# GBATZOLIS/ID-diff

Measured on AMD Instinct MI355X. Metric: score-vector evals/sec (rows of S per second incl. the per-point spectrum), 32x32 ncsnpp, higher is better.
Workload: dtype f32 (3x3 convs: Winograd, fp32 transforms, contraction on pairs of fp16 values -- 22 significand bits, 3 products, fp32 accumulate (F(4,3) along the rows x 3 filter rows); 1x1/attention/dense contractions: fp32 operands split exactly into 3 bf16, 6 partial products, fp32 accumulate; the q/k/v projec

## Files before the change

id-diff_amd/_lib.py:

```python
import ctypes
import os
import subprocess
from typing import NamedTuple, Optional

import torch

_HERE = os.path.dirname(os.path.abspath(__file__))
_VARIANT = os.environ.get("IDIFF_LIB_VARIANT", "")
_LIB_PATH = os.path.join(_HERE, "csrc", f"libidiff_hip.{_VARIANT}.so" if _VARIANT else "libidiff_hip.so")
_lib = None

ACT = {None: 0, "none": 0, "linear": 0, "silu": 1, "swish": 1, "elu": 2, "relu": 3, "lrelu": 4}

c_i, c_i64, c_f, c_d, c_p = ctypes.c_int, ctypes.c_int64, ctypes.c_float, ctypes.c_double, ctypes.c_void_p


class Epilogue(ctypes.Structure):
    _fields_ = [("bias", c_p), ("rowbias", c_p), ("ld_rowbias", c_i64), ("rows_per_group", c_i), ("act", c_i),
                ("residual", c_p), ("ld_residual", c_i64), ("out_scale", c_f), ("rowscale", c_p), ("colstats", c_p)]


_SIGNATURES = {
    "idiff_abi_version": (c_i, []),
    "idiff_last_error": (ctypes.c_char_p, []),
    "idiff_source_stamp": (ctypes.c_char_p, []),
    "idiff_variant_flags": (ctypes.c_char_p, []),
    "idiff_set_option": (c_i, [ctypes.c_char_p, c_i]),
    "idiff_gemm_pairs_ok": (c_i, [c_i, c_i, c_i, c_i]),
    "idiff_gemm_pairs_scale_f32": (c_i, [c_p, c_i64, c_i, c_i, c_p, c_p]),
    "idiff_gemm_pairs_f32": (c_i, [c_p, c_i64, c_i64, c_p, c_i64, c_i64, c_p, c_i, c_p, c_p, c_i64, c_i64, c_i, c_i, c_i, c_i, c_p, c_p]),
    "idiff_pairs_act_scale_f32": (c_i, [c_p, c_i, c_i, c_p, c_i, c_i, c_i, c_i, c_p, c_p]),
    "idiff_gemm_pairs_2src_f32": (c_i, [c_p, c_p, c_i64, c_i, c_p, c_p, c_i64, c_p, c_p, c_i64, c_i, c_i, c_i, c_p, c_p]),
    "idiff_set_thread_option": (c_i, [ctypes.c_char_p, c_i, c_i]),
    "idiff_upfirdn2d_f32": (c_i, [c_p, c_p, c_p] + [c_i] * 14 + [c_p]),
    "idiff_upfirdn2d_route": (ctypes.c_char_p, [c_p, c_p] + [c_i] * 14),
    "idiff_upfirdn2d_gn_f32": (c_i, [c_p, c_p, c_p, c_i, c_p] + [c_i] * 14 + [c_p]),
    "idiff_upfirdn2d_gn_ok": (c_i, [c_p, c_p, c_i, c_p] + [c_i] * 14),
    "idiff_fused_bias_act_f32": (c_i, [c_p, c_p, c_p, c_p, c_i64, c_i, c_i, c_i, c_i, c_f, c_f, c_p]),
    "idiff_upfirdn2d_f16": (c_i, [c_p, c_p, c_p] + [c_i] * 14 + [c_p]),
    "idiff_upfirdn2d_f64": (c_i, [c_p, c_p, c_p] + [c_i] * 14 + [c_p]),
    "idiff_fused_bias_act_f16": (c_i, [c_p, c_p, c_p, c_p, c_i64, c_i, c_i, c_i, c_i, c_f, c_f, c_p]),
    "idiff_fused_bias_act_f64": (c_i, [c_p, c_p, c_p, c_p, c_i64, c_i, c_i, c_i, c_i, c_f, c_f, c_p]),
    "idiff_gemm_f32": (c_i, [c_p, c_i64, c_i64, c_p, c_i64, c_i64, c_p, c_i64, c_i64, c_i, c_i, c_i, c_i,
                             ctypes.POINTER(Epilogue), c_p]),
    "idiff_gemm_2src_f32": (c_i, [c_p, c_p, c_i64, c_i, c_p, c_i64, c_p, c_i64, c_i, c_i, c_i, ctypes.POINTER(Epilogue), c_p]),
    "idiff_conv2d_nhwc_f32": (c_i, [c_p, c_p, c_p] + [c_i] * 10 + [ctypes.POINTER(Epilogue), c_p]),
    "idiff_gemm_route": (ctypes.c_char_p, [c_p, c_i64, c_i64, c_p, c_i64, c_i64, c_p, c_i64, c_i64, c_i, c_i, c_i, c_i,
                                           ctypes.POINTER(Epilogue), c_i]),
    "idiff_conv2d_route": (ctypes.c_char_p, [c_p, c_p, c_p] + [c_i] * 10 + [ctypes.POINTER(Epilogue)]),
    "idiff_gemm_colstats_split": (c_i, [c_i, c_i, c_i, c_i64, c_i64, c_i]),
    "idiff_conv2d_colstats_split": (c_i, [c_i] * 10),
    "idiff_conv2d_winograd_ok": (c_i, [c_i] * 5),
    "idiff_winograd_weight_floats": (c_i64, [c_i, c_i]),
    "idiff_winograd_pack_f32": (c_i, [c_p, c_p, c_i, c_i, c_p]),
    "idiff_conv2d_winograd_f32": (c_i, [c_p, c_p, c_p] + [c_i] * 5 + [ctypes.POINTER(Epilogue), c_p]),
    "idiff_conv2d_winograd_colstats_split": (c_i, [c_i] * 5),
    "idiff_conv2d_winograd43_ok": (c_i, [c_i] * 5),
    "idiff_conv2d_winograd43_colstats_split": (c_i, [c_i] * 5),
    "idiff_winograd43_weight_floats": (c_i64, [c_i, c_i]),
    "idiff_winograd43_pack_f32": (c_i, [c_p, c_p, c_i, c_i, c_p]),
    "idiff_conv2d_winograd43_f32": (c_i, [c_p, c_p, c_p, c_i, c_i, c_i, c_i, c_i, ctypes.POINTER(Epilogue), c_p]),
    "idiff_conv2d_winograd43h_ok": (c_i, [c_i] * 5),
    "idiff_winograd43h_weight_floats": (c_i64, [c_i, c_i]),
    "idiff_winograd43h_pack_f32": (c_i, [c_p, c_p, c_i, c_i, c_p]),
    "idiff_conv2d_winograd43h_f32": (c_i, [c_p, c_p, c_p, c_i, c_i, c_i, c_i, c_i, ctypes.POINTER(Epilogue), c_p]),
    "idiff_conv2d_wino1d_ok": (c_i, [c_i] * 5),
    "idiff_conv2d_wino1d_colstats_split": (c_i, [c_i] * 5),
    "idiff_wino1d_weight_floats": (c_i64, [c_i, c_i]),
    "idiff_wino1d_pack_f32": (c_i, [c_p, c_p, c_i, c_i, c_p]),
    "idiff_conv2d_wino1d_f32": (c_i, [c_p, c_p, c_p, c_i, c_i, c_i, c_i, c_i, ctypes.POINTER(Epilogue), c_p]),
    "idiff_conv2d_wino1d_gn_ok": (c_i, [c_i] * 6),
    "idiff_conv2d_wino1d_normload_ok": (c_i, [c_i] * 5),
    "idiff_conv2d_wino1d_normload_f32": (c_i, [c_p, c_p, c_p, c_i, c_i, c_i, c_i, c_i, ctypes.POINTER(Epilogue), c_p, c_i, c_p]),
    "idiff_conv2d_wino1d_normload_2src_ok": (c_i, [c_i] * 6),
    "idiff_conv2d_wino1d_normload_2src_f32": (c_i, [c_p, c_i, c_p, c_i, c_p, c_p, c_i, c_i, c_i, c_i, ctypes.POINTER(Epilogue), c_p, c_i, c_p]),
    "idiff_groupnorm_coef_f32": (c_i, [c_p, c_i, c_i, c_p, c_i, c_i, c_i, c_i, c_i, c_f, c_p, c_p, c_p, c_p]),
    "idiff_conv2d_wino1d_gn_f32": (c_i, [c_p, c_p, c_p, c_i, c_i, c_i, c_i, c_i, ctypes.POINTER(Epilogue), c_i, c_p, c_p, c_f, c_i, c_p]),
    "idiff_conv2d_winograd_split_ok": (c_i, [c_i] * 5),
    "idiff_winograd_split_weight_floats": (c_i64, [c_i, c_i]),
    "idiff_winograd_pack_split_f32": (c_i, [c_p, c_p, c_i, c_i, c_p]),
    "idiff_conv2d_winograd_split_f32": (c_i, [c_p, c_p, c_p] + [c_i] * 5 + [ctypes.POINTER(Epilogue), c_p]),
    "idiff_groupnorm_finalize_f32": (c_i, [c_p, c_i, c_i, c_p, c_i, c_i, c_i, c_i, c_i, c_f, c_p, c_p]),
    "idiff_groupnorm_nsplit": (c_i, [c_i, c_i, c_i]),
    "idiff_groupnorm_stats_f32": (c_i, [c_p, c_i, c_p, c_i, c_i, c_i, c_i, c_f, c_p, c_p, c_p]),
    "idiff_groupnorm_apply_f32": (c_i, [c_p, c_i, c_p, c_i, c_i, c_i, c_i, c_p, c_p, c_p, c_p, c_i64, c_i, c_p, c_p]),
    "idiff_groupnorm_apply_colstats_f32": (c_i, [c_p, c_i, c_p, c_i, c_i, c_i, c_i, c_p, c_i, c_p, c_i, c_f, c_p, c_p, c_p, c_i64,
                                                 c_i, c_p, c_p]),
    "idiff_groupnorm_apply_route": (ctypes.c_char_p, [c_p, c_i, c_p, c_i, c_i, c_i, c_i, c_p, c_p, c_p, c_p]),
    "idiff_groupnorm_apply_colstats_route": (ctypes.c_char_p, [c_p, c_i, c_p, c_i, c_i, c_i, c_i, c_p, c_i, c_p, c_i, c_p, c_p, c_p]),
    "idiff_softmax_rows_f32": (c_i, [c_p, c_p, c_i64, c_i, c_f, c_p]),
    "idiff_softmax_rows_route": (ctypes.c_char_p, [c_p, c_p, c_i64, c_i, c_f]),
    "idiff_attention256_ok": (c_i, [c_i, c_i, c_i]),
    "idiff_attention256_f32": (c_i, [c_p, c_i64, c_p, c_p, c_p, c_p, c_p, c_i, c_i, c_i, c_f, c_p]),
    "idiff_attention_heads_ok": (c_i, [c_i, c_i, c_i, c_i]),
    "idiff_attention_heads_f32": (c_i, [c_p, c_i64, c_p, c_p, c_p, c_p, c_p, c_i, c_i, c_i, c_i, c_f, c_p]),
    "idiff_attention256_route": (ctypes.c_char_p, [c_p, c_i64, c_p, c_p, c_p, c_p, c_p, c_i, c_i, c_i]),
    "idiff_attention_heads_route": (ctypes.c_char_p, [c_p, c_i64, c_p, c_p, c_p, c_p, c_p, c_i, c_i, c_i, c_i]),
    "idiff_affine_act_f32": (c_i, [c_p, c_p, c_i64, c_f, c_f, c_i, c_p, c_i64, c_p]),
    "idiff_add_scale_f32": (c_i, [c_p, c_p, c_p, c_i64, c_f, c_p]),
    "idiff_affine_act_route": (ctypes.c_char_p, [c_p, c_p, c_i64, c_p, c_i64]),
    "idiff_add_scale_route": (ctypes.c_char_p, [c_p, c_p, c_p, c_i64]),
    "idiff_concat_cols_route": (ctypes.c_char_p, [c_p, c_i, c_p, c_i, c_p, c_i64]),
    "idiff_fourier_embed_f32": (c_i, [c_p, c_p, c_p, c_i, c_i, c_p]),
    "idiff_positional_embed_f32": (c_i, [c_p, c_p, c_i, c_i, c_f, c_i, c_p]),
    "idiff_concat_cols_f32": (c_i, [c_p, c_i, c_p, c_i, c_p, c_i64, c_p]),
    "idiff_nchw_to_nhwc_f32": (c_i, [c_p, c_p, c_i, c_i, c_i, c_i, c_f, c_f, c_p]),
    "idiff_nhwc_to_nchw_f32": (c_i, [c_p, c_p, c_i, c_i, c_i, c_i, c_p, c_p]),
    "idiff_resample2x_nhwc_f32": (c_i, [c_p, c_p, c_i, c_i, c_i, c_i, c_i, c_p]),
    "idiff_perturb_f32": (c_i, [c_p, c_p, c_p, c_p, c_p, c_i64, c_i64, c_p]),
    "idiff_perturb_randn_f32": (c_i, [c_p, c_p, c_p, c_p, c_i64, c_i64, c_i64, ctypes.c_uint64, c_p, c_p]),
    "idiff_spectrum_workspace_bytes": (c_i64, [c_i, c_i, c_i]),
    "idiff_spectrum_f32": (c_i, [c_p, c_i, c_i, c_i, c_p, c_i64, c_p, c_p, c_p]),
    "idiff_colmean_f64": (c_i, [c_p, c_i, c_i, c_i, c_p, c_p, c_p]),
    "idiff_centered_gram_f64": (c_i, [c_p, c_p, c_i, c_i, c_i, c_p, c_p]),
    "idiff_centered_gram_rows_f64": (c_i, [c_p, c_p, c_i, c_i, c_i, c_i, c_p, c_p]),
    "idiff_symmetrize_upper_f64": (c_i, [c_p, c_i, c_p]),
    "idiff_symtridiag_scratch_doubles": (c_i64, [c_i]),
    "idiff_symband_ld": (c_i, []),
    "idiff_symband_f64": (c_i, [c_p, c_i, c_p, c_p]),
    "idiff_symtridiag_f64": (c_i, [c_p, c_i, c_i, c_p, c_p, c_p, c_p]),
    "idiff_symtridiag_plan": (c_i, [c_i]),
    "idiff_tridiag_eigvals_f64": (c_i, [c_p, c_p, c_i, c_i, c_p, c_p]),
    "idiff_sym_lowvecs_scratch_doubles": (c_i64, [c_i, c_i]),
    "idiff_sym_lowvecs_f64": (c_i, [c_p, c_i, c_i, c_p, c_p, c_p, c_p, c_p]),
    "idiff_sym_topvecs_scratch_doubles": (c_i64, [c_i, c_i, c_i]),
    "idiff_sym_topvecs_f64": (c_i, [c_p, c_i, c_i, c_i, c_d, c_d, c_d, c_i, c_i, c_p, c_p, c_p, c_p, c_p]),
    "idiff_knn_workspace_bytes": (c_i64, [c_i, c_i, c_i]),
    "idiff_knn_f32": (c_i, [c_p, c_i, c_i, c_i, c_p, c_i64, c_p, c_p, c_p, c_p]),
# ... 300 lines not shown
def gemm_pairs_ok(M, N, K, batch=1):
    return bool(lib().idiff_gemm_pairs_ok(M, N, K, batch))


def gemm_pairs_scale(w):
    _dev(w, "w")
    out = torch.empty(2, device=w.device, dtype=torch.float32)
    _check(lib().idiff_gemm_pairs_scale_f32(w.data_ptr(), w.stride(0), w.shape[0], w.shape[1], out.data_ptr(), _stream()),
           "idiff_gemm_pairs_scale_f32")
    return out


def gemm_pairs(a, bt, w_scale, out, epilogue=None, weight_is_a=False, M=None, N=None, K=None, lda=None, ldb=None, ldc=None,
               batch=1, stride_a=0, stride_b=0, stride_c=0, act_scale=None):
    explicit = M is not None
    _dev(a, "a", contiguous=not explicit); _dev(bt, "bt", contiguous=not explicit); _dev(out, "out", contiguous=not explicit)
    _dev(w_scale, "w_scale")
    if M is None:
        M, K = a.shape
        N = bt.shape[0]
        if bt.shape[1] != K or out.shape[0] != M or out.shape[1] != N:
            raise RuntimeError(f"gemm_pairs: shapes {tuple(a.shape)} x {tuple(bt.shape)}^T -> {tuple(out.shape)}")
        lda, ldb, ldc = a.stride(0), bt.stride(0), out.stride(0)
    ep = _ep_ref(epilogue, "gemm_pairs")
    _check(lib().idiff_gemm_pairs_f32(a.data_ptr(), lda, stride_a, bt.data_ptr(), ldb, stride_b, w_scale.data_ptr(), int(bool(weight_is_a)),
                                      _ptr(act_scale), out.data_ptr(), ldc, stride_c, M, N, K, batch, ep, _stream()), "idiff_gemm_pairs_f32")
    return out


def pairs_act_scale(stats1, C1, stats2, C2, B, HW):
    out = torch.empty(8, device=stats1[0].device, dtype=torch.float32)
    _check(lib().idiff_pairs_act_scale_f32(stats1[0].data_ptr(), stats1[1], C1, _ptr(stats2[0]) if stats2 is not None else None,
                                           stats2[1] if stats2 is not None else 0, C2, B, HW, out.data_ptr(), _stream()),
           "idiff_pairs_act_scale_f32")
    return out


def gemm_pairs_2src(a1, a2, act_scale, bt, w_scale, out, epilogue=None):
    _dev(a1, "a1"); _dev(a2, "a2"); _dev(bt, "bt"); _dev(out, "out"); _dev(act_scale, "act_scale"); _dev(w_scale, "w_scale")
    M, K1 = a1.shape
    K = K1 + a2.shape[1]
    if a2.shape[0] != M or a1.stride(0) != a2.stride(0) or bt.shape[1] != K:
        raise RuntimeError(f"gemm_pairs_2src: shapes {tuple(a1.shape)} | {tuple(a2.shape)} x {tuple(bt.shape)}^T")
    ep = _ep_ref(epilogue, "gemm_pairs_2src")
    _check(lib().idiff_gemm_pairs_2src_f32(a1.data_ptr(), a2.data_ptr(), a1.stride(0), K1, act_scale.data_ptr(), bt.data_ptr(), bt.stride(0),
                                           w_scale.data_ptr(), out.data_ptr(), out.stride(0), M, bt.shape[0], K, ep, _stream()),
           "idiff_gemm_pairs_2src_f32")
    return out


def gemm_normed(cache, a, w, out, epilogue=None, pairs=True):
    M, K = a.shape
    if not pairs or not gemm_pairs_ok(M, w.shape[0], K):
        return gemm(a, w, out=out, epilogue=epilogue)
    return gemm_pairs(a, w, _pairs_scale_of(cache, w), out, epilogue=epilogue)


def _pairs_scale_of(cache, w):
    sc = cache.setdefault("pairs_scale", {})
    if id(w) not in sc:
        sc[id(w)] = (gemm_pairs_scale(w), w)
    return sc[id(w)][0]


def gemm_weight_times_normed_t(cache, w, x, out, B, HW, C, pairs=True):
    kw = dict(M=C, N=HW, K=C, lda=C, ldb=C, ldc=HW, batch=B, stride_a=0, stride_b=HW * C, stride_c=C * HW)
    if not pairs or not gemm_pairs_ok(C, HW, C, B):
        return gemm(w, x, out=out, **kw)
    return gemm_pairs(w, x, _pairs_scale_of(cache, w), out, weight_is_a=True, **kw)


def gemm_2src(a1, a2, bt, out, epilogue=None):
    _dev(a1, "a1"); _dev(a2, "a2"); _dev(bt, "bt"); _dev(out, "out")
    M, K1 = a1.shape
    K = K1 + a2.shape[1]
    if a2.shape[0] != M or a1.stride(0) != a2.stride(0) or bt.shape[1] != K:
        raise RuntimeError(f"gemm_2src: shapes {tuple(a1.shape)} | {tuple(a2.shape)} x {tuple(bt.shape)}^T")
    ep = _ep_ref(epilogue, "gemm_2src")
    _check(lib().idiff_gemm_2src_f32(a1.data_ptr(), a2.data_ptr(), a1.stride(0), K1, bt.data_ptr(), bt.stride(0), out.data_ptr(),
                                     out.stride(0), M, bt.shape[0], K, ep, _stream()), "idiff_gemm_2src_f32")
    return out


def conv2d_nhwc(x, wt, out, B, H, W, Cin, Cout, KH, KW, stride, pad, epilogue=None, pad_hi=None):
    ep = _ep_ref(epilogue, "conv2d_nhwc")
    _check(lib().idiff_conv2d_nhwc_f32(x.data_ptr(), wt.data_ptr(), out.data_ptr(), B, H, W, Cin, Cout, KH, KW, stride,
                                       pad, pad if pad_hi is None else pad_hi, ep, _stream()), "idiff_conv2d_nhwc_f32")
    return out


def _addr(t):
    return t if isinstance(t, int) else t.data_ptr()


def gemm_route(a, bt, out, M, N, K, lda, ldb, ldc, epilogue=None, batch=1, stride_a=0, stride_b=0, stride_c=0, pairs=False):
    name = lib().idiff_gemm_route(_addr(a), lda, stride_a, _addr(bt), ldb, stride_b, _addr(out), ldc, stride_c, M, N, K, batch,
                                  _ep_ref(epilogue, "gemm_route"), int(bool(pairs)))
    return None if name is None else name.decode()


def conv2d_route(x, wt, out, B, H, W, Cin, Cout, KH, KW, stride, pad, epilogue=None, pad_hi=None):
    name = lib().idiff_conv2d_route(_addr(x), _addr(wt), _addr(out), B, H, W, Cin, Cout, KH, KW, stride, pad, pad if pad_hi is None else pad_hi,
                                    _ep_ref(epilogue, "conv2d_route"))
    return None if name is None else name.decode()


def _wino_pack(stem, name, wt, Cin, Cout):
    _dev(wt, "wt")
    if tuple(wt.shape) != (Cout, 3, 3, Cin):
        raise RuntimeError(f"{name}: expected {Cout}x3x3x{Cin} weights, got {tuple(wt.shape)}")
    entry = "idiff_winograd_pack_split_f32" if stem == "winograd_split" else f"idiff_{stem}_pack_f32"
    u = torch.empty(getattr(lib(), f"idiff_{stem}_weight_floats")(Cin, Cout), device=wt.device, dtype=torch.float32)
    _check(getattr(lib(), entry)(wt.data_ptr(), u.data_ptr(), Cin, Cout, _stream()), entry)
    return u


def _wino_conv(stem, packed_by, x, u, out, B, H, W, Cin, Cout, epilogue):
    want = getattr(lib(), f"idiff_{stem}_weight_floats")(Cin, Cout)
    if u.numel() != want:
        raise RuntimeError(f"conv2d_{stem}: a filter bank of {u.numel()} floats ({want} expected): pack it with {packed_by}")
    gn = getattr(epilogue, "groupnorm", None)
    nl = getattr(epilogue, "normload", None)
    if nl is not None and stem == "wino1d":
        if gn is not None:
            raise RuntimeError("conv2d_wino1d: a GroupNorm in the loader (with_normload) and one in the tail (with_groupnorm) in one launch")
        if nl.coef.numel() != B * Cin * 2:
            raise RuntimeError(f"conv2d_wino1d: {nl.coef.numel()} loader coefficients for [B, Cin, 2] = [{B}, {Cin}, 2]")
        if nl.x2 is not None:
            _check(lib().idiff_conv2d_wino1d_normload_2src_f32(x.data_ptr(), nl.C1, nl.x2.data_ptr(), Cin - nl.C1, u.data_ptr(), out.data_ptr(),
                                                               B, H, W, Cout, ctypes.byref(epilogue), nl.coef.data_ptr(), nl.act, _stream()),
                   "idiff_conv2d_wino1d_normload_2src_f32")
        else:
            _check(lib().idiff_conv2d_wino1d_normload_f32(x.data_ptr(), u.data_ptr(), out.data_ptr(), B, H, W, Cin, Cout, ctypes.byref(epilogue),
                                                          nl.coef.data_ptr(), nl.act, _stream()), "idiff_conv2d_wino1d_normload_f32")
        return out
    if gn is not None and stem == "wino1d":
        groups, gamma, beta, eps, act = gn
        if gamma.numel() != Cout or beta.numel() != Cout:
            raise RuntimeError(f"conv2d_wino1d: fused GroupNorm with {gamma.numel()} / {beta.numel()} gamma / beta entries for {Cout} channels")
        _check(lib().idiff_conv2d_wino1d_gn_f32(x.data_ptr(), u.data_ptr(), out.data_ptr(), B, H, W, Cin, Cout, ctypes.byref(epilogue), groups,
                                                gamma.data_ptr(), beta.data_ptr(), eps, act, _stream()), "idiff_conv2d_wino1d_gn_f32")
        return out
    ep = _ep_ref(epilogue, f"conv2d_{stem}")
    entry = f"idiff_conv2d_{stem}_f32"
    _check(getattr(lib(), entry)(x.data_ptr(), u.data_ptr(), out.data_ptr(), B, H, W, Cin, Cout, ep, _stream()), entry)
    return out


def conv2d_winograd_ok(B, H, W, Cin, Cout):
    return bool(lib().idiff_conv2d_winograd_ok(B, H, W, Cin, Cout))


def conv2d_winograd_split_ok(B, H, W, Cin, Cout):
    return bool(lib().idiff_conv2d_winograd_split_ok(B, H, W, Cin, Cout))


def conv2d_winograd_colstats_split(B, H, W, Cin, Cout):
    return lib().idiff_conv2d_winograd_colstats_split(B, H, W, Cin, Cout)


def winograd_pack(wt, Cin, Cout, split=False):
    return _wino_pack("winograd_split" if split else "winograd", "winograd_pack", wt, Cin, Cout)


def conv2d_winograd(x, u, out, B, H, W, Cin, Cout, epilogue=None, split=False):
    return _wino_conv("winograd_split" if split else "winograd", f"winograd_pack(..., split={split})", x, u, out, B, H, W, Cin, Cout, epilogue)
# ... 1308 lines not shown
```

id-diff_amd/csrc/common.h:

```cpp
#pragma once
#include <hip/hip_runtime.h>
#include <stdint.h>
#include <stdio.h>
#include <stdarg.h>

#include "../../include/idiff_hip.h"

#define IDIFF_API extern "C" __attribute__((visibility("default")))

namespace idiff {

void set_error(const char *fmt, ...);

inline int fail(const char *fmt, ...) {
  char buf[512];
  va_list ap;
  va_start(ap, fmt);
  vsnprintf(buf, sizeof(buf), fmt, ap);
  va_end(ap);
  set_error("%s", buf);
  return IDIFF_EINVAL;
}

inline int launch_status(const char *what) {
  hipError_t e = hipGetLastError();
  if (e != hipSuccess) {
    set_error("%s: %s", what, hipGetErrorString(e));
    return (int)e;
  }
  return 0;
}

enum Option { OPT_NO_WINOGRAD, OPT_NO_COLSTATS, OPT_NO_PIPE, OPT_SCALAR_EPILOGUE, OPT_DBUF_ONLY, OPT_TRIDIAG_ONESTAGE,
              OPT_UFD_ROWS, OPT_CHASE_WAVEFRONT, OPT_WINO_NGROUP, OPT_GRAM_SMALL_TILES, OPT_CHASE_SPIN_LIMIT, OPT_FAKE_CU_COUNT,
              OPT_SBR_SYNC, OPT_SBR_FULL, OPT_NO_SPLIT, OPT_WINO_SPLIT, OPT_SBR_LOOKAHEAD, OPT_NO_WINO43, OPT_NO_WINO43H, OPT_NO_PAIRS, OPT_PAIRS_MIN_TILES, OPT_NO_FUSED_ATTN, OPT_NO_WINO1D, OPT_NO_FUSED_GN, OPT_NO_FUSED_GN_LOAD, OPT_NO_FUSED_GN_LOAD_2SRC, OPT_NO_FUSED_GN_FIR, OPT_COUNT };
bool option(Option o);
int option_value(Option o);

struct AttrGuard { unsigned long long done_mask = 0; };
int set_dynamic_lds_once(AttrGuard &g, const void *const *fns, int n_fns, int bytes, const char *what);

bool conv3x3_narrow_ok(int B, int H, int W, int Cin, int Cout, int KH, int KW, int stride, int pad_lo, int pad_hi,
                       const idiff_epilogue *ep);
int conv3x3_narrow(const float *x, const float *wt, float *out, int B, int H, int W, int Cin, int Cout,
                   const idiff_epilogue *ep, hipStream_t stream);

template <class P> inline void set_epilogue(P &p, const idiff_epilogue *ep) {
  p.has_ep = ep ? 1 : 0;
  p.ep = ep ? *ep : idiff_epilogue{};
  if (!ep) p.ep.out_scale = 1.f;
  if (p.ep.rows_per_group <= 0) p.ep.rows_per_group = 1;
}

inline idiff_epilogue shift_epilogue(const idiff_epilogue &ep, int64_t m0) {
  idiff_epilogue e = ep;
  const int64_t g0 = m0 / (ep.rows_per_group > 0 ? ep.rows_per_group : 1);
  if (e.rowbias) e.rowbias += g0 * ep.ld_rowbias;
  if (e.residual) e.residual += m0 * ep.ld_residual;
  if (e.rowscale) e.rowscale += g0;
  return e;
}
inline int64_t host_cut_row(int64_t units, int64_t unit_rows, const idiff_epilogue *ep) {
  const int64_t rpg = (ep && ep->rows_per_group > 0) ? ep->rows_per_group : 1;
  const int64_t half = units / 2 * unit_rows;
  return unit_rows == 1 ? half / rpg * rpg : half % rpg ? 0 : half;
}
template <class Run> inline int run_cut(int64_t rows, int64_t cut, const idiff_epilogue *ep, bool first_only, Run run) {
  if (int rc = run((int64_t)0, cut, ep)) return rc;
  if (first_only) return 0;
  idiff_epilogue hi;
  if (ep) hi = shift_epilogue(*ep, cut);
  return run(cut, rows, ep ? &hi : nullptr);
}

static inline int ceil_div(int a, int b) { return (a + b - 1) / b; }
static inline int64_t ceil_div64(int64_t a, int64_t b) { return (a + b - 1) / b; }

static inline int streaming_grid(int64_t work_items, int block) {
  int64_t g = ceil_div64(work_items, block);
  const int64_t cap = 256 * 8;
  if (g > cap) g = cap;
  if (g < 1) g = 1;
  return (int)g;
}

__device__ __forceinline__ float act_apply(float v, int act) {
  switch (act) {
    case IDIFF_ACT_SILU: return v * __frcp_rn(1.0f + __expf(-v));
    case IDIFF_ACT_ELU: return v > 0.f ? v : (expf(v) - 1.0f);
    case IDIFF_ACT_RELU: return v > 0.f ? v : 0.f;
    case IDIFF_ACT_LRELU: return v > 0.f ? v : 0.2f * v;
    default: return v;
  }
}

}
```

id-diff_amd/csrc/igemm.hip:

```cpp
#include "common.h"
#include <type_traits>
#include <stdlib.h>

namespace {

typedef float floatx16 __attribute__((ext_vector_type(16)));

constexpr int BK = 32;
constexpr int LDS_PITCH = BK + 4;

struct IgemmParams {
  const float *A;
  const float *Bt;
  float *C;
  int64_t lda, ldb, ldc;
  int64_t strideA, strideB, strideC;
  int M, N, K;
  int tiles_m, tiles_n;
  int H, W, Cin, OH, OW, KW, stride, pad;
  idiff_epilogue ep;
  int has_ep;
  uint32_t a_bytes, b_bytes;
  int vec_ep;
  const float *A2;
  int K1;
  uint32_t a2_bytes;
  uint32_t c_bytes, res_bytes;
  int buf_ep;
  const float *scale_a, *scale_b;
};

__device__ __forceinline__ float4 ldg4(const float *p) { return *reinterpret_cast<const float4 *>(p); }

template <int BM, int BN, int WARPS_M, int WARPS_N, bool CONV, bool VEC>
__global__ void __launch_bounds__(WARPS_M *WARPS_N * 64)
igemm_kernel(const IgemmParams p) {
  constexpr int T = WARPS_M * WARPS_N * 64;
  constexpr int WTM = BM / WARPS_M, WTN = BN / WARPS_N;
  constexpr int TM = WTM / 32, TN = WTN / 32;
  constexpr int A_PER_T = BM * (BK / 4) / T;
  constexpr int B_PER_T = BN * (BK / 4) / T;
  static_assert(A_PER_T >= 1 && B_PER_T >= 1, "tile too small for the thread count");
  static_assert(T % (BK / 4) == 0, "a thread keeps one k-column of float4s");

  extern __shared__ __attribute__((aligned(16))) float lds[];
  float *As = lds;
  float *Bs = lds + 2 * BM * LDS_PITCH;

  const int nwg = p.tiles_m * p.tiles_n;
  int bid = blockIdx.x;
  {
    const int q = nwg >> 3, r = nwg & 7, xcd = bid & 7, local = bid >> 3;
    bid = (xcd < r ? xcd * (q + 1) : r * (q + 1) + (xcd - r) * q) + local;
  }
  const int tile_n = bid % p.tiles_n, tile_m = bid / p.tiles_n;
  const int batch = blockIdx.y;
  const int m0 = tile_m * BM, n0 = tile_n * BN;

  const int tid = threadIdx.x, lane = tid & 63, wave = tid >> 6;
  const int wm0 = (wave / WARPS_N) * WTM, wn0 = (wave % WARPS_N) * WTN;

  const float *Ab = p.A + (int64_t)batch * p.strideA;
  const float *Bb = p.Bt + (int64_t)batch * p.strideB;

  const int kc = (tid & 7) * 4;
  const int row_base = tid >> 3;
  constexpr int ROW_STEP = T / 8;

  int64_t a_off[A_PER_T];
  int a_iy[A_PER_T], a_ix[A_PER_T];
  bool a_ok[A_PER_T];
#pragma unroll
  for (int i = 0; i < A_PER_T; ++i) {
    const int m = m0 + row_base + i * ROW_STEP;
    a_ok[i] = m < p.M;
    if (CONV) {
      const int mm = a_ok[i] ? m : 0;
      const int ox = mm % p.OW;
      const int t = mm / p.OW;
      const int oy = t % p.OH;
      const int b = t / p.OH;
      a_off[i] = (int64_t)b * p.H * p.W;
      a_iy[i] = oy * p.stride - p.pad;
      a_ix[i] = ox * p.stride - p.pad;
    } else {
      a_off[i] = (int64_t)m * p.lda;
      a_iy[i] = a_ix[i] = 0;
    }
  }
  int64_t b_off[B_PER_T];
  bool b_ok[B_PER_T];
#pragma unroll
  for (int i = 0; i < B_PER_T; ++i) {
    const int n = n0 + row_base + i * ROW_STEP;
    b_ok[i] = n < p.N;
    b_off[i] = (int64_t)n * p.ldb;
  }

  float4 a_reg[A_PER_T], b_reg[B_PER_T];

  auto load_scalar4 = [&](const float *base, int k, bool ok) -> float4 {
    float4 v = make_float4(0.f, 0.f, 0.f, 0.f);
    if (ok) {
      if (k + 0 < p.K) v.x = base[0];
      if (k + 1 < p.K) v.y = base[1];
      if (k + 2 < p.K) v.z = base[2];
      if (k + 3 < p.K) v.w = base[3];
    }
    return v;
  };

  auto fetch = [&](int kt) {
// ... 78 lines not shown
  const idiff_epilogue &ep = p.ep;
  const int col_l = lane & 31, row_l = (lane >> 5) * 4;
#pragma unroll
  for (int j = 0; j < TN; ++j) {
    const int n = n0 + wn0 + j * 32 + col_l;
    if (n >= p.N) continue;
    const float bias = (p.has_ep && ep.bias) ? ep.bias[n] : 0.f;
#pragma unroll
    for (int i = 0; i < TM; ++i) {
#pragma unroll
      for (int r = 0; r < 16; ++r) {
        const int m = m0 + wm0 + i * 32 + (r & 3) + 8 * (r >> 2) + row_l;
        if (m >= p.M) continue;
        float v = acc[i][j][r] + bias;
        if (p.has_ep) {
          if (ep.rowbias) v += ep.rowbias[(int64_t)(m / ep.rows_per_group) * ep.ld_rowbias + n];
          v = idiff::act_apply(v, ep.act);
          if (ep.residual) v += ep.residual[(int64_t)m * ep.ld_residual + n];
          v *= ep.out_scale;
          if (ep.rowscale) v *= ep.rowscale[m / ep.rows_per_group];
        }
        Cb[(int64_t)m * p.ldc + n] = v;
      }
    }
  }
}

template <int BM, int BN, int WARPS_M, int WARPS_N, bool CONV, bool VEC>
int launch_cfg(IgemmParams &p, int batch, hipStream_t st) {
  p.tiles_m = idiff::ceil_div(p.M, BM);
  p.tiles_n = idiff::ceil_div(p.N, BN);
  constexpr size_t lds_bytes = (size_t)2 * (BM + BN) * LDS_PITCH * sizeof(float);
  auto kern = igemm_kernel<BM, BN, WARPS_M, WARPS_N, CONV, VEC>;
  if (lds_bytes > 64 * 1024) {
    static idiff::AttrGuard guard;
    const void *fn = reinterpret_cast<const void *>(kern);
    if (int rc = idiff::set_dynamic_lds_once(guard, &fn, 1, (int)lds_bytes, "igemm")) return rc;
  }
  dim3 grid(p.tiles_m * p.tiles_n, batch);
  hipLaunchKernelGGL(kern, grid, dim3(WARPS_M * WARPS_N * 64), lds_bytes, st, p);
  return idiff::launch_status(CONV ? "igemm_conv" : "igemm_linear");
}


typedef unsigned int uintx4 __attribute__((ext_vector_type(4)));
typedef __bf16 bf16x8 __attribute__((ext_vector_type(8)));
constexpr uint32_t OOB = 0xFFFFFFFFu;

constexpr int SP = BK;
__device__ __forceinline__ int split_swz(int row) { return (row ^ (row >> 2)) & 3; }

__device__ __forceinline__ void split4(const float4 v, uint2 &p1, uint2 &p2, uint2 &p3) {
  const float x[4] = {v.x, v.y, v.z, v.w};
  uint32_t t1[4], t2[4], t3[4];
#pragma unroll
  for (int e = 0; e < 4; ++e) {
    t1[e] = __float_as_uint(x[e]) & 0xffff0000u;
    const float r1 = x[e] - __uint_as_float(t1[e]);
    t2[e] = __float_as_uint(r1) & 0xffff0000u;
    t3[e] = __float_as_uint(r1 - __uint_as_float(t2[e]));
  }
  p1 = make_uint2((t1[0] >> 16) | t1[1], (t1[2] >> 16) | t1[3]);
  p2 = make_uint2((t2[0] >> 16) | t2[1], (t2[2] >> 16) | t2[3]);
  p3 = make_uint2((t3[0] >> 16) | (t3[1] & 0xffff0000u), (t3[2] >> 16) | (t3[3] & 0xffff0000u));
}
typedef _Float16 halfx8 __attribute__((ext_vector_type(8)));
__device__ __forceinline__ void pair4(const float4 v, uint2 &hi, uint2 &lo) {
  typedef float f2 __attribute__((ext_vector_type(2)));
  typedef _Float16 h2 __attribute__((ext_vector_type(2)));
  const f2 v01 = {v.x, v.y}, v23 = {v.z, v.w};
  const h2 h01 = __builtin_convertvector(v01, h2), h23 = __builtin_convertvector(v23, h2);
  const f2 r01 = v01 - __builtin_convertvector(h01, f2), r23 = v23 - __builtin_convertvector(h23, f2);
  const h2 l01 = __builtin_convertvector(r01, h2), l23 = __builtin_convertvector(r23, h2);
  hi = make_uint2(__builtin_bit_cast(uint32_t, h01), __builtin_bit_cast(uint32_t, h23));
  lo = make_uint2(__builtin_bit_cast(uint32_t, l01), __builtin_bit_cast(uint32_t, l23));
}
bool aligned16(const void *ptr) { return ((uintptr_t)ptr & 15) == 0; }

__device__ __forceinline__ float4 buf_load4(__amdgpu_buffer_rsrc_t r, uint32_t byte_off) {
  const uintx4 v = __builtin_amdgcn_raw_buffer_load_b128(r, (int)byte_off, 0, 0);
  return __builtin_bit_cast(float4, v);
}

template <int BM, int BN, int WARPS_M, int WARPS_N, bool CONV, bool DBUF, int SPLIT>
__global__ void __launch_bounds__(WARPS_M *WARPS_N * 64, (DBUF || SPLIT) ? 2 : 4)
igemm_pipe_kernel(const IgemmParams p) {
  static_assert(!(SPLIT && DBUF), "the split form uses one LDS buffer");
  constexpr int T = WARPS_M * WARPS_N * 64;
  constexpr int WTM = BM / WARPS_M, WTN = BN / WARPS_N;
  constexpr int TM = WTM / 32, TN = WTN / 32;
  constexpr int A_PER_T = BM * (BK / 4) / T;
  constexpr int B_PER_T = BN * (BK / 4) / T;
  constexpr int ROW_STEP = T / 8;

  extern __shared__ __attribute__((aligned(16))) float lds[];
  float *As = lds;
  float *Bs = lds + (DBUF ? 2 : 1) * BM * LDS_PITCH;
  constexpr int PLANES = SPLIT == 2 ? 2 : 3;
  unsigned short *As16 = reinterpret_cast<unsigned short *>(lds);
  unsigned short *Bs16 = As16 + (DBUF ? 2 : 1) * PLANES * BM * SP;

  const int nwg = p.tiles_m * p.tiles_n;
  int bid = blockIdx.x;
  {
    const int q = nwg >> 3, r = nwg & 7, xcd = bid & 7, local = bid >> 3;
    bid = (xcd < r ? xcd * (q + 1) : r * (q + 1) + (xcd - r) * q) + local;
  }
  const int tile_n = bid % p.tiles_n, tile_m = bid / p.tiles_n;
  const int batch = blockIdx.y;
  const int m0 = tile_m * BM, n0 = tile_n * BN;
  const int tid = threadIdx.x, lane = tid & 63, wave = tid >> 6;
  const int wm0 = (wave / WARPS_N) * WTM, wn0 = (wave % WARPS_N) * WTN;

  const __amdgpu_buffer_rsrc_t rA =
      __builtin_amdgcn_make_buffer_rsrc((void *)(p.A + (int64_t)batch * p.strideA), 0, (int)p.a_bytes, 0x00020000);
  const __amdgpu_buffer_rsrc_t rB =
      __builtin_amdgcn_make_buffer_rsrc((void *)(p.Bt + (int64_t)batch * p.strideB), 0, (int)p.b_bytes, 0x00020000);
  const __amdgpu_buffer_rsrc_t rA2 =
      __builtin_amdgcn_make_buffer_rsrc((void *)(p.K1 > 0 ? p.A2 : p.A), 0, (int)(p.K1 > 0 ? p.a2_bytes : p.a_bytes), 0x00020000);

  const int kc = (tid & 7) * 4;
  const int row_base = tid >> 3;

  uint32_t a_base[A_PER_T], a_mask[A_PER_T];
#pragma unroll
  for (int i = 0; i < A_PER_T; ++i) {
    const int m = m0 + row_base + i * ROW_STEP;
    const bool ok = m < p.M;
    if (CONV) {
      const int mm = ok ? m : 0;
      const int ox = mm % p.OW;
      const int t = mm / p.OW;
      const int oy = t % p.OH;
      const int b = t / p.OH;
      const int iy0 = oy * p.stride - p.pad, ix0 = ox * p.stride - p.pad;
      a_base[i] = (uint32_t)(((b * p.H + iy0) * p.W + ix0) * p.Cin + kc) * 4u;
      uint32_t mask = 0;
      const int KH = p.K / (p.KW * p.Cin);
      for (int ky = 0; ky < KH; ++ky)
        for (int kx = 0; kx < p.KW; ++kx) {
          const int iy = iy0 + ky, ix = ix0 + kx;
          if (ok && iy >= 0 && iy < p.H && ix >= 0 && ix < p.W) mask |= 1u << (ky * p.KW + kx);
        }
      a_mask[i] = mask;
    } else {
      a_base[i] = (uint32_t)((int64_t)m * p.lda + kc) * 4u;
      a_mask[i] = ok ? 1u : 0u;
    }
  }
  uint32_t b_base[B_PER_T];
  bool b_ok[B_PER_T];
#pragma unroll
  for (int i = 0; i < B_PER_T; ++i) {
    const int n = n0 + row_base + i * ROW_STEP;
    b_ok[i] = n < p.N;
    b_base[i] = (uint32_t)((int64_t)n * p.ldb + kc) * 4u;
  }

  float4 a_reg[A_PER_T], b_reg[B_PER_T];
  int f_kt = 0, f_c0 = 0, f_tap = 0, f_ky = 0, f_kx = 0;

  const int ntaps = CONV ? p.K / p.Cin : 1;
  auto fetch = [&]() {
    const int k = f_kt * BK + kc;
    const bool kok = k < p.K;
    uint32_t koffb = (uint32_t)f_kt * (BK * 4u);
    if (CONV && p.Cin == 4) {
      const int tap = f_kt * 8 + (tid & 7);
      const int ky = tap / p.KW, kx = tap - ky * p.KW;
      const uint32_t tapoff = (uint32_t)((ky * p.W + kx) * 4 - kc) * 4u;
#pragma unroll
      for (int i = 0; i < A_PER_T; ++i) {
        const bool ok = tap < ntaps && ((a_mask[i] >> tap) & 1u);
        a_reg[i] = buf_load4(rA, ok ? a_base[i] + tapoff : OOB);
      }
    } else if (CONV) {
      const uint32_t tapoff = (uint32_t)((f_ky * p.W + f_kx) * p.Cin + f_c0) * 4u;
      koffb = (uint32_t)(f_tap * p.Cin + f_c0) * 4u;
#pragma unroll
      for (int i = 0; i < A_PER_T; ++i) {
        const bool ok = (a_mask[i] >> f_tap) & 1u;
        a_reg[i] = buf_load4(rA, ok ? a_base[i] + tapoff : OOB);
      }
      ++f_tap;
      if (++f_kx == p.KW) { f_kx = 0; ++f_ky; }
      if (f_tap == ntaps) { f_tap = 0; f_kx = 0; f_ky = 0; f_c0 += BK; }
    } else {
      const bool second = p.K1 > 0 && f_kt * BK >= p.K1;
      const __amdgpu_buffer_rsrc_t rS = second ? rA2 : rA;
      const uint32_t koff = (uint32_t)(f_kt * BK - (second ? p.K1 : 0)) * 4u;
#pragma unroll
      for (int i = 0; i < A_PER_T; ++i) a_reg[i] = buf_load4(rS, (a_mask[i] && kok) ? a_base[i] + koff : OOB);
    }
#pragma unroll
    for (int i = 0; i < B_PER_T; ++i) b_reg[i] = buf_load4(rB, (b_ok[i] && kok) ? b_base[i] + koffb : OOB);
    ++f_kt;
  };

  static_assert(ROW_STEP % 16 == 0 && BM % 32 == 0 && BN % 32 == 0, "split-plane swizzle");
  const int kc_sw = (((kc >> 3) ^ split_swz(row_base)) << 3) + (kc & 7);
  const float pair_sa = (SPLIT == 2 && p.scale_a) ? p.scale_a[0] : 1.f, pair_s = (SPLIT == 2 && p.scale_b) ? p.scale_b[0] : 1.f;
  auto stage = [&](int buf) {
    if (SPLIT == 2) {
      unsigned short *a_dst = As16, *b_dst = Bs16;
#pragma unroll
      for (int i = 0; i < A_PER_T; ++i) {
        uint2 hi, lo;
        const float4 av = a_reg[i];
        pair4(make_float4(av.x * pair_sa, av.y * pair_sa, av.z * pair_sa, av.w * pair_sa), hi, lo);
        unsigned short *d = a_dst + (row_base + i * ROW_STEP) * SP + kc_sw;
        *reinterpret_cast<uint2 *>(d) = hi;
        *reinterpret_cast<uint2 *>(d + BM * SP) = lo;
      }
#pragma unroll
      for (int i = 0; i < B_PER_T; ++i) {
        uint2 hi, lo;
        const float4 w = b_reg[i];
        pair4(make_float4(w.x * pair_s, w.y * pair_s, w.z * pair_s, w.w * pair_s), hi, lo);
        unsigned short *d = b_dst + (row_base + i * ROW_STEP) * SP + kc_sw;
        *reinterpret_cast<uint2 *>(d) = hi;
        *reinterpret_cast<uint2 *>(d + BN * SP) = lo;
      }
      return;
    }
    if (SPLIT) {
      unsigned short *a_dst = As16 + buf * 3 * BM * SP, *b_dst = Bs16 + buf * 3 * BN * SP;
#pragma unroll
      for (int i = 0; i < A_PER_T; ++i) {
        uint2 q1, q2, q3;
        split4(a_reg[i], q1, q2, q3);
        unsigned short *d = a_dst + (row_base + i * ROW_STEP) * SP + kc_sw;
        *reinterpret_cast<uint2 *>(d) = q1;
        *reinterpret_cast<uint2 *>(d + BM * SP) = q2;
        *reinterpret_cast<uint2 *>(d + 2 * BM * SP) = q3;
      }
#pragma unroll
      for (int i = 0; i < B_PER_T; ++i) {
        uint2 q1, q2, q3;
        split4(b_reg[i], q1, q2, q3);
        unsigned short *d = b_dst + (row_base + i * ROW_STEP) * SP + kc_sw;
        *reinterpret_cast<uint2 *>(d) = q1;
        *reinterpret_cast<uint2 *>(d + BN * SP) = q2;
        *reinterpret_cast<uint2 *>(d + 2 * BN * SP) = q3;
      }
      return;
    }
    float *a_dst = As + buf * BM * LDS_PITCH;
    float *b_dst = Bs + buf * BN * LDS_PITCH;
#pragma unroll
    for (int i = 0; i < A_PER_T; ++i)
      *reinterpret_cast<float4 *>(a_dst + (row_base + i * ROW_STEP) * LDS_PITCH + kc) = a_reg[i];
#pragma unroll
    for (int i = 0; i < B_PER_T; ++i)
      *reinterpret_cast<float4 *>(b_dst + (row_base + i * ROW_STEP) * LDS_PITCH + kc) = b_reg[i];
  };

  floatx16 acc[TM][TN];

  const int frag_row = lane & 31, frag_k = (lane >> 5) * 4;
  const int nkt = (p.K + BK - 1) / BK;

  fetch();
  stage(0);
  if (nkt > 1) fetch();
  __syncthreads();

  auto ktile = [&](int kt, auto first) {
    const int buf = DBUF ? (kt & 1) : 0;
    if (DBUF && !SPLIT) {
      if (kt + 1 < nkt) stage(buf ^ 1);
      if (kt + 2 < nkt) fetch();
    }
    if (SPLIT == 2) {
      const int c0 = (lane >> 5) ^ split_swz(frag_row);
      const unsigned short *a16 = As16 + (wm0 + frag_row) * SP, *b16 = Bs16 + (wn0 + frag_row) * SP;
// ... 239 lines not shown
            const float4 rb = *reinterpret_cast<const float4 *>(ep.rowbias + (int64_t)grp * ep.ld_rowbias + n);
            v[0] += rb.x; v[1] += rb.y; v[2] += rb.z; v[3] += rb.w;
          }
#pragma unroll
          for (int e = 0; e < 4; ++e) v[e] = idiff::act_apply(v[e], ep.act);
          if (ep.residual) {
            const float4 rs = *reinterpret_cast<const float4 *>(ep.residual + (int64_t)m * ep.ld_residual + n);
            v[0] += rs.x; v[1] += rs.y; v[2] += rs.z; v[3] += rs.w;
          }
          const float rsc = ep.rowscale ? ep.rowscale[grp] : 1.f;
#pragma unroll
          for (int e = 0; e < 4; ++e) { v[e] *= ep.out_scale; if (ep.rowscale) v[e] *= rsc; }
        }
        *reinterpret_cast<float4 *>(Cb + (int64_t)m * p.ldc + n) = make_float4(v[0], v[1], v[2], v[3]);
        if (want_stats) {
#pragma unroll
          for (int e = 0; e < 4; ++e) { s1[e] += (double)v[e]; s2[e] += (double)v[e] * (double)v[e]; }
        }
      }
    }
    if (want_stats) {
#pragma unroll
      for (int off = C4; off < 64; off <<= 1)
#pragma unroll
        for (int e = 0; e < 4; ++e) { s1[e] += __shfl_xor(s1[e], off, 64); s2[e] += __shfl_xor(s2[e], off, 64); }
      __syncthreads();
      if (lane < C4) {
#pragma unroll
        for (int e = 0; e < 4; ++e) {
          const int slot = ((wave / WARPS_N) * BN + wn0 + c4 * 4 + e) * 2;
          red[slot] = s1[e]; red[slot + 1] = s2[e];
        }
      }
    }
  } else {
#pragma unroll
  for (int j = 0; j < TN; ++j) {
    const int n = n0 + wn0 + j * 32 + col_l;
    const bool n_ok = n < p.N;
    const float bias = (n_ok && p.has_ep && ep.bias) ? ep.bias[n] : 0.f;
    double s1 = 0.0, s2 = 0.0;
#pragma unroll
    for (int i = 0; i < TM; ++i) {
#pragma unroll
      for (int r = 0; r < 16; ++r) {
        const int m = m0 + wm0 + i * 32 + (r & 3) + 8 * (r >> 2) + row_l;
        if (m >= p.M || !n_ok) continue;
        float v = acc[i][j][r] + bias;
        if (p.has_ep) {
          if (ep.rowbias) v += ep.rowbias[(int64_t)(m / ep.rows_per_group) * ep.ld_rowbias + n];
          v = idiff::act_apply(v, ep.act);
          if (ep.residual) v += ep.residual[(int64_t)m * ep.ld_residual + n];
          v *= ep.out_scale;
          if (ep.rowscale) v *= ep.rowscale[m / ep.rows_per_group];
        }
        Cb[(int64_t)m * p.ldc + n] = v;
        if (want_stats) { s1 += (double)v; s2 += (double)v * (double)v; }
      }
    }
    if (want_stats) {
      s1 += __shfl_xor(s1, 32, 64);
      s2 += __shfl_xor(s2, 32, 64);
      if (lane < 32) {
        const int slot = ((wave / WARPS_N) * BN + wn0 + j * 32 + col_l) * 2;
        red[slot] = s1; red[slot + 1] = s2;
      }
    }
  }
  }
  if (want_stats) {
    __syncthreads();
    for (int c = tid; c < BN; c += T) {
      const int n = n0 + c;
      if (n >= p.N) continue;
      double a = 0.0, b = 0.0;
#pragma unroll
      for (int w = 0; w < WARPS_M; ++w) { a += red[(w * BN + c) * 2]; b += red[(w * BN + c) * 2 + 1]; }
      double *dst = ep.colstats + ((int64_t)tile_m * p.N + n) * 2;
      dst[0] = a; dst[1] = b;
    }
  }
}

template <int BM, int BN, int WARPS_M, int WARPS_N, bool CONV, bool DBUF = true, int SPLIT = 0>
int launch_pipe(IgemmParams &p, int batch, hipStream_t st) {
  p.tiles_m = idiff::ceil_div(p.M, BM);
  p.tiles_n = idiff::ceil_div(p.N, BN);
  constexpr size_t stage_bytes = SPLIT ? (size_t)(DBUF ? 2 : 1) * (BM + BN) * (SPLIT == 2 ? 2 : 3) * SP * sizeof(unsigned short)
                                       : (size_t)(DBUF ? 2 : 1) * (BM + BN) * LDS_PITCH * sizeof(float);
  constexpr size_t patch_bytes = (size_t)WARPS_M * WARPS_N * 32 * (BN / WARPS_N) * sizeof(float);
  constexpr size_t lds_bytes = stage_bytes > patch_bytes ? stage_bytes : patch_bytes;
  auto kern = igemm_pipe_kernel<BM, BN, WARPS_M, WARPS_N, CONV, DBUF, SPLIT>;
  if (lds_bytes > 64 * 1024) {
    static idiff::AttrGuard guard;
    const void *fn = reinterpret_cast<const void *>(kern);
    if (int rc = idiff::set_dynamic_lds_once(guard, &fn, 1, (int)lds_bytes, "igemm")) return rc;
  }
  dim3 grid(p.tiles_m * p.tiles_n, batch);
  hipLaunchKernelGGL(kern, grid, dim3(WARPS_M * WARPS_N * 64), lds_bytes, st, p);
  return idiff::launch_status(CONV ? "igemm_pipe_conv" : "igemm_pipe_linear");
}

enum IgemmFamily { FAM_PIPE, FAM_DIRECT_VEC, FAM_DIRECT_SCALAR, FAM_NARROW };
enum IgemmArith { AR_FP32, AR_FP32_1BUF, AR_SPLIT, AR_PAIRS };
enum IgemmEpForm { EPF_BUF_BLOCK, EPF_BUF_ROW, EPF_VEC64, EPF_SCALAR };
struct IgemmPlan { int family, bm, bn, arith, ep_form; };
enum IgemmWant { WANT_PIPE, WANT_PAIRS, WANT_DIRECT_VEC, WANT_DIRECT_SCALAR };

constexpr int64_t BUF_LIMIT = 0xFFFFFFF0ll;
int64_t extent_bytes(int64_t rows, int64_t ld, int64_t row_len) { return ((rows - 1) * ld + row_len) * 4; }

IgemmPlan igemm_tile(int M, int N, int batch, int want) {
  IgemmPlan c = {};
  const int64_t wg_big = (int64_t)idiff::ceil_div(M, 128) * idiff::ceil_div(N, 128) * batch;
  const int64_t wg_mid = (int64_t)idiff::ceil_div(M, 128) * idiff::ceil_div(N, 64) * batch;
  auto tile = [&](int bm, int bn, int arith) { c.bm = bm; c.bn = bn; c.arith = arith; };
  c.ep_form = EPF_SCALAR;
  if (want == WANT_DIRECT_VEC || want == WANT_DIRECT_SCALAR) {
    c.family = want == WANT_DIRECT_VEC ? FAM_DIRECT_VEC : FAM_DIRECT_SCALAR;
    if (N > 64 && wg_big >= 256) tile(128, 128, AR_FP32);
    else if (wg_mid >= 256 || M >= 4096) tile(128, 64, AR_FP32);
    else tile(64, 64, AR_FP32);
    return c;
  }
  c.family = FAM_PIPE;
  if (want == WANT_PAIRS) tile(128, 128, AR_PAIRS);
  else if (!idiff::option(idiff::OPT_NO_SPLIT)) {
    if (N > 64 && wg_big >= 256) tile(128, 128, AR_SPLIT);
    else if (N <= 32 && M >= 4096) tile(128, 32, AR_SPLIT);
    else if (wg_mid >= 256 || M >= 4096) tile(128, 64, AR_SPLIT);
    else tile(64, 64, AR_SPLIT);
  }
  else if (N > 64 && wg_big >= 1024 && !idiff::option(idiff::OPT_DBUF_ONLY)) tile(128, 128, AR_FP32_1BUF);
  else if (N > 64 && wg_big >= 256) tile(128, 128, AR_FP32);
  else if (N <= 32 && M >= 4096) tile(128, 32, AR_FP32);
  else if (wg_mid >= 256 || M >= 4096) tile(128, 64, AR_FP32);
  else tile(64, 64, AR_FP32);
  return c;
}

IgemmPlan igemm_choose(IgemmParams &p, int batch, int want) {
  IgemmPlan c = igemm_tile(p.M, p.N, batch, want);
  if (c.family != FAM_PIPE) return c;
  const idiff_epilogue &e = p.ep;
  const bool al = (p.N % 4 == 0) && (p.ldc % 4 == 0) && (p.strideC % 4 == 0) && aligned16(p.C) &&
                  (!p.has_ep || ((!e.bias || aligned16(e.bias)) && (!e.rowbias || (aligned16(e.rowbias) && e.ld_rowbias % 4 == 0)) &&
                                 (!e.residual || (aligned16(e.residual) && e.ld_residual % 4 == 0))));
  p.vec_ep = al && !idiff::option(idiff::OPT_SCALAR_EPILOGUE);
  const int64_t c_bytes = extent_bytes(p.M, p.ldc, p.N);
  const int64_t res_bytes = (p.has_ep && e.residual) ? extent_bytes(p.M, e.ld_residual, p.N) : 0;
  const int64_t pitch = p.ldc > e.ld_residual ? p.ldc : e.ld_residual;
  p.buf_ep = p.vec_ep && c_bytes < 0xE0000000ll && res_bytes < 0xE0000000ll && (int64_t)c.bm * pitch * 4 < 0x0FFFFFF0ll;
  p.c_bytes = p.buf_ep ? (uint32_t)c_bytes : 0; p.res_bytes = p.buf_ep ? (uint32_t)res_bytes : 0;
  c.ep_form = !p.vec_ep ? EPF_SCALAR : !p.buf_ep ? EPF_VEC64 : (e.rows_per_group % 32 == 0 ? EPF_BUF_BLOCK : EPF_BUF_ROW);
  return c;
}

template <bool CONV>
int igemm_launch(const IgemmPlan &c, IgemmParams &p, int batch, hipStream_t st) {
  const int t = c.bm * 1000 + c.bn;
  if (c.family == FAM_DIRECT_VEC || c.family == FAM_DIRECT_SCALAR) {
    const bool vec = c.family == FAM_DIRECT_VEC;
    if constexpr (CONV) {
      if (vec && t == 128128) return launch_cfg<128, 128, 2, 2, true, true>(p, batch, st);
      if (vec && t == 128064) return launch_cfg<128, 64, 2, 2, true, true>(p, batch, st);
      if (vec && t == 64064) return launch_cfg<64, 64, 2, 2, true, true>(p, batch, st);
    } else {
      if (t == 128128) return vec ? launch_cfg<128, 128, 2, 2, false, true>(p, batch, st) : launch_cfg<128, 128, 2, 2, false, false>(p, batch, st);
      if (t == 128064) return vec ? launch_cfg<128, 64, 2, 2, false, true>(p, batch, st) : launch_cfg<128, 64, 2, 2, false, false>(p, batch, st);
      if (t == 64064) return vec ? launch_cfg<64, 64, 2, 2, false, true>(p, batch, st) : launch_cfg<64, 64, 2, 2, false, false>(p, batch, st);
    }
  } else if (c.family == FAM_PIPE) {
    switch (c.arith) {
      case AR_PAIRS:
        if constexpr (!CONV) { if (t == 128128) return launch_pipe<128, 128, 2, 2, false, false, 2>(p, batch, st); }
        break;
      case AR_SPLIT:
        if (t == 128128) return launch_pipe<128, 128, 2, 2, CONV, false, 1>(p, batch, st);
        if (t == 128032) return launch_pipe<128, 32, 4, 1, CONV, false, 1>(p, batch, st);
        if (t == 128064) return launch_pipe<128, 64, 2, 2, CONV, false, 1>(p, batch, st);
        if (t == 64064) return launch_pipe<64, 64, 2, 2, CONV, false, 1>(p, batch, st);
        break;
      case AR_FP32_1BUF:
        if (t == 128128) return launch_pipe<128, 128, 2, 2, CONV, false>(p, batch, st);
        break;
      case AR_FP32:
        if (t == 128128) return launch_pipe<128, 128, 2, 2, CONV>(p, batch, st);
        if (t == 128032) return launch_pipe<128, 32, 4, 1, CONV>(p, batch, st);
        if (t == 128064) return launch_pipe<128, 64, 2, 2, CONV>(p, batch, st);
        if (t == 64064) return launch_pipe<64, 64, 2, 2, CONV>(p, batch, st);
        break;
    }
  }
  return idiff::fail("igemm: no kernel for the plan (family %d, tile %d x %d, arithmetic %d)", c.family, c.bm, c.bn, c.arith);
}

const char *igemm_plan_name(const IgemmPlan &c) {
  static const char *const fam[] = {"pipe", "direct-vec", "direct-scalar", "narrow"};
  static const char *const ar[] = {"fp32", "fp32-1buf", "split", "pairs"};
  static const char *const epf[] = {"buf-block", "buf-row", "vec64", "scalar"};
  static thread_local char text[64];
  if (c.family == FAM_NARROW) snprintf(text, sizeof(text), "narrow c%d fp32 %s", c.bn, c.ep_form == 2 ? "elem" : c.ep_form == 1 ? "row" : "none");
  else snprintf(text, sizeof(text), "%s %dx%d %s %s", fam[c.family], c.bm, c.bn, ar[c.arith], epf[c.ep_form]);
  return text;
}

template <bool CONV>
int igemm_run(IgemmParams &p, int batch, int want, hipStream_t st, IgemmPlan *probe) {
  const IgemmPlan c = igemm_choose(p, batch, want);
  if (p.has_ep && p.ep.colstats && c.family == FAM_PIPE && p.M % c.bm)
    return idiff::fail("%s: colstats with M = %d rows in tiles of %d: no whole tiles (ask idiff_%s_colstats_split first)", CONV ? "conv2d" : "gemm",
                       p.M, c.bm, CONV ? "conv2d" : "gemm");
  if (probe) { *probe = c; return 0; }
  return igemm_launch<CONV>(c, p, batch, st);
}

enum PipeServes { PIPE_NO, PIPE_YES, PIPE_A_BEYOND };
bool pitches16(int K, int64_t lda, int64_t ldb) { return K % 4 == 0 && lda % 4 == 0 && ldb % 4 == 0; }
int pipe_fits_linear(int M, int N, int K, int64_t lda, int64_t ldb, int K1 = 0) {
  if (!pitches16(K, lda, ldb) || extent_bytes(N, ldb, K) >= BUF_LIMIT) return PIPE_NO;
  return extent_bytes(M, lda, K1 > K - K1 ? K1 : K - K1) < BUF_LIMIT ? PIPE_YES : PIPE_A_BEYOND;
}
int pipe_serves_linear(int M, int N, int K, int64_t lda, int64_t ldb, int K1 = 0) {
  return idiff::option(idiff::OPT_NO_PIPE) ? PIPE_NO : pipe_fits_linear(M, N, K, lda, ldb, K1);
}
int pipe_serves_conv(int B, int H, int W, int Cin, int Cout, int KH, int KW) {
  const int64_t K = (int64_t)KH * KW * Cin;
  if ((Cin % BK && Cin != 4) || KH * KW > 32 || idiff::option(idiff::OPT_NO_PIPE) || extent_bytes(Cout, K, K) >= BUF_LIMIT) return PIPE_NO;
  return extent_bytes((int64_t)B * H * W, Cin, Cin) < BUF_LIMIT ? PIPE_YES : PIPE_A_BEYOND;
}

IgemmParams igemm_params(const float *A, int64_t lda, const float *Bt, int64_t ldb, float *C, int64_t ldc, int M, int N, int K,
                         const idiff_epilogue *ep) {
  IgemmParams p = {};
  p.A = A; p.Bt = Bt; p.C = C; p.lda = lda; p.ldb = ldb; p.ldc = ldc; p.M = M; p.N = N; p.K = K;
  idiff::set_epilogue(p, ep);
  return p;
}

__global__ void __launch_bounds__(256) pairs_scale_kernel(const float *__restrict__ bt, int64_t ldb, int N, int K, float *__restrict__ out) {
  __shared__ float red[256];
  float m = 0.f;
  for (int64_t i = threadIdx.x; i < (int64_t)N * K; i += 256) m = fmaxf(m, fabsf(bt[(i / K) * ldb + (i % K)]));
  red[threadIdx.x] = m;
  __syncthreads();
  for (int off = 128; off > 0; off >>= 1) {
    if ((int)threadIdx.x < off) red[threadIdx.x] = fmaxf(red[threadIdx.x], red[threadIdx.x + off]);
    __syncthreads();
  }
  if (threadIdx.x == 0) {
    const float mx = red[0];
    int e = 0;
    if (mx > 0.f && mx < INFINITY) (void)frexpf(mx, &e);
    const int sh = mx > 0.f && mx < INFINITY ? 12 - e : 0;
    out[0] = ldexpf(1.f, sh);
    out[1] = ldexpf(1.f, -sh);
  }
}
bool pairs_geometry_ok(int M, int N, int K, int batch) {
  if (M <= 0 || N <= 64 || K <= 0 || K % 4 || batch <= 0 || batch > 65535) return false;
  const int want = idiff::option_value(idiff::OPT_PAIRS_MIN_TILES);
  return (int64_t)idiff::ceil_div(M, 128) * idiff::ceil_div(N, 128) * batch >= (want > 0 ? want : 256);
}
}

IDIFF_API int idiff_gemm_pairs_ok(int M, int N, int K, int batch) {
  if (idiff::option(idiff::OPT_NO_PIPE) || idiff::option(idiff::OPT_NO_SPLIT) || idiff::option(idiff::OPT_NO_PAIRS)) return 0;
  return pairs_geometry_ok(M, N, K, batch) ? 1 : 0;
}

IDIFF_API int idiff_gemm_pairs_scale_f32(const float *Bt, int64_t ldb, int N, int K, float *scale, void *stream) {
  using namespace idiff;
  if (!Bt || !scale) return fail("gemm_pairs_scale: null pointer");
  if (N <= 0 || K <= 0 || ldb < K) return fail("gemm_pairs_scale: bad shape N=%d K=%d ldb=%lld", N, K, (long long)ldb);
  hipLaunchKernelGGL(pairs_scale_kernel, dim3(1), dim3(256), 0, (hipStream_t)stream, Bt, ldb, N, K, scale);
  return launch_status("gemm_pairs_scale");
}

namespace {
__global__ void __launch_bounds__(256) pairs_act_scale_kernel(const double *__restrict__ ws1, int64_t n1, const double *__restrict__ ws2,
                                                              int64_t n2, double count, float *__restrict__ out) {
  __shared__ double red[256];
  double acc = 0.0;
  const int64_t stride = (int64_t)gridDim.x * 256;
  for (int64_t i = (int64_t)blockIdx.x * 256 + threadIdx.x; i < n1; i += stride) acc += ws1[2 * i + 1];
  for (int64_t i = (int64_t)blockIdx.x * 256 + threadIdx.x; i < n2; i += stride) acc += ws2[2 * i + 1];
  red[threadIdx.x] = acc;
  __syncthreads();
  for (int off = 128; off > 0; off >>= 1) {
    if ((int)threadIdx.x < off) red[threadIdx.x] += red[threadIdx.x + off];
    __syncthreads();
  }
  if (threadIdx.x == 0) {
    double *total = reinterpret_cast<double *>(out + 2);
    unsigned int *done = reinterpret_cast<unsigned int *>(out + 4);
    atomicAdd(total, red[0]);
    __threadfence();
    if (atomicAdd(done, 1u) == gridDim.x - 1) {
      __threadfence();
      const double ms = *reinterpret_cast<volatile double *>(total) / count;
      int sh = 0;
      if (ms > 0.0 && ms < 1e300) {
        int e = 0;
        (void)frexp(sqrt(ms), &e);
        sh = -e + ((sqrt(ms) * ldexp(1.0, -e) < 0.70710678118654752) ? 1 : 0);
      }
      out[0] = ldexpf(1.f, sh);
      out[1] = ldexpf(1.f, -sh);
    }
  }
}
}

IDIFF_API int idiff_pairs_act_scale_f32(const double *ws1, int nsplit1, int C1, const double *ws2, int nsplit2, int C2, int B, int HW,
                                        float *out, void *stream) {
  using namespace idiff;
  if (!ws1 || !out || nsplit1 <= 0 || C1 <= 0 || B <= 0 || HW <= 0 || (ws2 && (nsplit2 <= 0 || C2 <= 0)))
    return fail("pairs_act_scale: bad arguments");
  const int64_t n1 = (int64_t)B * nsplit1 * C1, n2 = ws2 ? (int64_t)B * nsplit2 * C2 : 0;
  hipError_t e = hipMemsetAsync(out, 0, 32, (hipStream_t)stream);
  if (e != hipSuccess) return fail("pairs_act_scale: hipMemsetAsync: %s", hipGetErrorString(e));
  const int blocks = (int)std::min<int64_t>(512, (n1 + n2 + 255) / 256);
  hipLaunchKernelGGL(pairs_act_scale_kernel, dim3(blocks), dim3(256), 0, (hipStream_t)stream, ws1, n1, ws2, n2,
                     (double)B * HW * (C1 + (ws2 ? C2 : 0)), out);
  return launch_status("pairs_act_scale");
}

namespace {
struct LinearCall {
  const char *name;
  const float *A, *A2;
  int K1;
  bool two_src;
  const float *Bt;
  float *C;
  int64_t lda, ldb, ldc, strideA, strideB, strideC;
  int M, N, K, batch;
  const idiff_epilogue *ep;
  int want;
  const float *w_scale, *act_scale;
  int weight_is_a;
};

int linear_front(const LinearCall &c, hipStream_t st, IgemmPlan *probe) {
  using namespace idiff;
  const bool pairs = c.want == WANT_PAIRS, colstats = c.ep && c.ep->colstats;
  if (c.M < 0 || c.N < 0 || c.K <= 0 || c.batch < 0 || (c.two_src && (c.K1 <= 0 || c.K1 >= c.K)))
    return c.two_src ? fail("%s: bad sizes M=%d N=%d K=%d K1=%d", c.name, c.M, c.N, c.K, c.K1)
                     : fail("%s: bad sizes M=%d N=%d K=%d batch=%d", c.name, c.M, c.N, c.K, c.batch);
  if (c.M == 0 || c.N == 0 || c.batch == 0) { if (probe) probe->family = -1; return 0; }
  if (!c.A || (c.two_src && !c.A2) || !c.Bt || !c.C || (pairs && !c.w_scale)) return fail("%s: null pointer", c.name);
  if (c.K1 % BK) return fail("%s: the split column K1 = %d must be a multiple of %d", c.name, c.K1, BK);
  if (c.lda < c.K1 || c.lda < c.K - c.K1 || c.ldb < c.K || c.ldc < c.N) return fail("%s: leading dimension smaller than the row length", c.name);
  if (pairs && !pairs_geometry_ok(c.M, c.N, c.K, c.batch))
    return fail("%s: M=%d N=%d K=%d batch=%d not served (ask idiff_gemm_pairs_ok)", c.name, c.M, c.N, c.K, c.batch);
  if (c.batch > 65535) return fail("%s: batch %d exceeds grid.y", c.name, c.batch);
  const bool vec = pitches16(c.K, c.lda, c.ldb) && c.strideA % 4 == 0 && c.strideB % 4 == 0 && aligned16(c.A) &&
                   (!c.two_src || aligned16(c.A2)) && aligned16(c.Bt);
  const int serves = !vec ? PIPE_NO : (pairs ? pipe_fits_linear : pipe_serves_linear)(c.M, c.N, c.K, c.lda, c.ldb, c.K1);
  if (serves == PIPE_A_BEYOND && c.batch == 1 && !pairs) {
    if (colstats) return fail("%s: colstats is not available for operands beyond 4 GiB", c.name);
    if (const int64_t cut = host_cut_row(c.M, 1, c.ep))
      return run_cut(c.M, cut, c.ep, probe != nullptr, [&](int64_t r0, int64_t r1, const idiff_epilogue *e) {
        LinearCall h = c;
        h.A += r0 * c.lda; h.C += r0 * c.ldc; h.M = (int)(r1 - r0); h.ep = e;
        if (c.two_src) h.A2 += r0 * c.lda;
        h.strideA = h.strideB = h.strideC = 0;
        return linear_front(h, st, probe);
      });
    if (c.two_src) return fail("%s: cannot split %d rows inside an epilogue row group of %d", c.name, c.M, c.ep ? c.ep->rows_per_group : 1);
  }
  IgemmParams p = igemm_params(c.A, c.lda, c.Bt, c.ldb, c.C, c.ldc, c.M, c.N, c.K, c.ep);
  p.strideA = c.strideA; p.strideB = c.strideB; p.strideC = c.strideC;
  if (serves != PIPE_YES) {
    if (pairs) return fail("%s: operands must be 16-byte aligned with row pitches and batch strides that are multiples of 4, one "
                           "batch slice inside 4 GiB", c.name);
    if (c.two_src) return fail("%s: operands must be 16-byte aligned with K %% 4 == 0 and lda %% 4 == 0 (use two idiff_gemm_f32 calls)", c.name);
    if (colstats) return fail("%s: colstats requested for a problem the pipelined kernel does not take "
                              "(ask idiff_gemm_colstats_split first)", c.name);
    return igemm_run<false>(p, c.batch, vec ? WANT_DIRECT_VEC : WANT_DIRECT_SCALAR, st, probe);
  }
  if (pairs && colstats && c.batch != 1) return fail("%s: colstats only for unbatched problems", c.name);
  p.a_bytes = (uint32_t)extent_bytes(c.M, c.lda, c.two_src ? c.K1 : c.K); p.b_bytes = (uint32_t)extent_bytes(c.N, c.ldb, c.K);
  if (c.two_src) { p.A2 = c.A2; p.K1 = c.K1; p.a2_bytes = (uint32_t)extent_bytes(c.M, c.lda, c.K - c.K1); }
  if (pairs) { p.scale_a = c.weight_is_a ? c.w_scale : c.act_scale; p.scale_b = c.weight_is_a ? c.act_scale : c.w_scale; }
  return igemm_run<false>(p, c.batch, c.want, st, probe);
}

LinearCall linear_call(const char *name, const float *A, int64_t lda, int64_t strideA, const float *Bt, int64_t ldb, int64_t strideB, float *C,
                       int64_t ldc, int64_t strideC, int M, int N, int K, int batch, const idiff_epilogue *ep, int want) {
  return LinearCall{name, A, nullptr, 0, false, Bt, C, lda, ldb, ldc, strideA, strideB, strideC, M, N, K, batch, ep, want, nullptr, nullptr, 0};
}
LinearCall linear_call_2src(const char *name, const float *A1, const float *A2, int64_t lda, int K1, const float *Bt, int64_t ldb, float *C,
                            int64_t ldc, int M, int N, int K, const idiff_epilogue *ep, int want) {
  LinearCall c = linear_call(name, A1, lda, 0, Bt, ldb, 0, C, ldc, 0, M, N, K, 1, ep, want);
  c.A2 = A2; c.K1 = K1; c.two_src = true;
  return c;
}
}

IDIFF_API int idiff_gemm_f32(const float *A, int64_t lda, int64_t strideA, const float *Bt, int64_t ldb,
                             int64_t strideB, float *C, int64_t ldc, int64_t strideC, int M, int N, int K,
                             int batch, const idiff_epilogue *ep, void *stream) {
  return linear_front(linear_call("gemm", A, lda, strideA, Bt, ldb, strideB, C, ldc, strideC, M, N, K, batch, ep, WANT_PIPE), (hipStream_t)stream,
                      nullptr);
}

IDIFF_API int idiff_gemm_pairs_f32(const float *A, int64_t lda, int64_t strideA, const float *Bt, int64_t ldb, int64_t strideB,
                                   const float *w_scale, int weight_is_a, const float *act_scale, float *C, int64_t ldc, int64_t strideC,
                                   int M, int N, int K, int batch, const idiff_epilogue *ep, void *stream) {
  LinearCall c = linear_call("gemm_pairs", A, lda, strideA, Bt, ldb, strideB, C, ldc, strideC, M, N, K, batch, ep, WANT_PAIRS);
  c.w_scale = w_scale; c.act_scale = act_scale; c.weight_is_a = weight_is_a;
  return linear_front(c, (hipStream_t)stream, nullptr);
}

IDIFF_API int idiff_gemm_2src_f32(const float *A1, const float *A2, int64_t lda, int K1, const float *Bt, int64_t ldb,
                                  float *C, int64_t ldc, int M, int N, int K, const idiff_epilogue *ep, void *stream) {
  return linear_front(linear_call_2src("gemm_2src", A1, A2, lda, K1, Bt, ldb, C, ldc, M, N, K, ep, WANT_PIPE), (hipStream_t)stream, nullptr);
}

IDIFF_API int idiff_gemm_pairs_2src_f32(const float *A1, const float *A2, int64_t lda, int K1, const float *act_scale, const float *Bt,
                                        int64_t ldb, const float *w_scale, float *C, int64_t ldc, int M, int N, int K,
                                        const idiff_epilogue *ep, void *stream) {
  LinearCall c = linear_call_2src("gemm_pairs_2src", A1, A2, lda, K1, Bt, ldb, C, ldc, M, N, K, ep, WANT_PAIRS);
  c.w_scale = w_scale; c.act_scale = act_scale;
  return linear_front(c, (hipStream_t)stream, nullptr);
}

IDIFF_API const char *idiff_gemm_route(const void *A, int64_t lda, int64_t strideA, const void *Bt, int64_t ldb, int64_t strideB,
                                       const void *C, int64_t ldc, int64_t strideC, int M, int N, int K, int batch,
                                       const idiff_epilogue *ep, int pairs) {
  IgemmPlan plan = {};
  LinearCall c = linear_call(pairs ? "gemm_pairs" : "gemm", (const float *)A, lda, strideA, (const float *)Bt, ldb, strideB,
                             (float *)const_cast<void *>(C), ldc, strideC, M, N, K, batch, ep, pairs ? WANT_PAIRS : WANT_PIPE);
  c.w_scale = c.Bt;
  if (linear_front(c, nullptr, &plan)) return nullptr;
  return plan.family < 0 ? "none" : igemm_plan_name(plan);
}

namespace {
int conv_front(const float *x, const float *wt, float *out, int B, int H, int W, int Cin, int Cout, int KH, int KW, int stride, int pad_lo,
               int pad_hi, const idiff_epilogue *ep, void *stream, IgemmPlan *probe) {
  using namespace idiff;
  if (B < 0 || H <= 0 || W <= 0 || Cin <= 0 || Cout <= 0 || KH <= 0 || KW <= 0 || stride <= 0 || pad_lo < 0 || pad_hi < 0)
    return fail("conv2d: bad geometry");
  if (Cin % 4 != 0) return fail("conv2d: Cin must be a multiple of 4 (pad the channels), got %d", Cin);
  if (B == 0) { if (probe) probe->family = -1; return 0; }
  if (!x || !wt || !out) return fail("conv2d: null pointer");
  if (!aligned16(x) || !aligned16(wt)) return fail("conv2d: x and wt must be 16-byte aligned");
  const int OH = (H + pad_lo + pad_hi - KH) / stride + 1, OW = (W + pad_lo + pad_hi - KW) / stride + 1;
  const int pad = pad_lo;
  if (H + pad_lo + pad_hi < KH || W + pad_lo + pad_hi < KW || OH <= 0 || OW <= 0) return fail("conv2d: empty output");
  const int64_t M64 = (int64_t)B * OH * OW;
  if (M64 > 0x7fffffff) return fail("conv2d: B*OH*OW overflows int32");
  if (conv3x3_narrow_ok(B, H, W, Cin, Cout, KH, KW, stride, pad_lo, pad_hi, ep)) {
    if (probe) {
      const int rpg = (ep && ep->rows_per_group > 0) ? ep->rows_per_group : 1;
      *probe = IgemmPlan{FAM_NARROW, 0, Cout, AR_FP32, !(ep && ep->rowscale) ? 0 : rpg % W == 0 ? 1 : 2};
      return 0;
    }
    return conv3x3_narrow(x, wt, out, B, H, W, Cin, Cout, ep, (hipStream_t)stream);
  }
  const int serves = pipe_serves_conv(B, H, W, Cin, Cout, KH, KW);
  if (ep && ep->colstats && serves != PIPE_YES)
    return fail("conv2d: colstats requested for a problem the pipelined kernel does not take "
                "(ask idiff_conv2d_colstats_split first)");
  if (serves == PIPE_A_BEYOND && B > 1) {
    if (const int64_t cut = host_cut_row(B, OH * OW, ep))
      return run_cut(M64, cut, ep, probe != nullptr, [&](int64_t r0, int64_t r1, const idiff_epilogue *e) {
        return conv_front(x + r0 / (OH * OW) * H * W * Cin, wt, out + r0 * Cout, (int)((r1 - r0) / (OH * OW)), H, W, Cin, Cout, KH, KW, stride,
                          pad_lo, pad_hi, e, stream, probe);
      });
  }
  const int K = KH * KW * Cin;
  IgemmParams p = igemm_params(x, 0, wt, K, out, Cout, (int)M64, Cout, K, ep);
  p.H = H; p.W = W; p.Cin = Cin; p.OH = OH; p.OW = OW; p.KW = KW; p.stride = stride; p.pad = pad;
  if (serves != PIPE_YES) return igemm_run<true>(p, 1, WANT_DIRECT_VEC, (hipStream_t)stream, probe);
  p.a_bytes = (uint32_t)extent_bytes((int64_t)B * H * W, Cin, Cin); p.b_bytes = (uint32_t)extent_bytes(Cout, K, K);
  return igemm_run<true>(p, 1, WANT_PIPE, (hipStream_t)stream, probe);
}
}

IDIFF_API int idiff_conv2d_nhwc_f32(const float *x, const float *wt, float *out, int B, int H, int W, int Cin,
                                    int Cout, int KH, int KW, int stride, int pad_lo, int pad_hi,
                                    const idiff_epilogue *ep, void *stream) {
  return conv_front(x, wt, out, B, H, W, Cin, Cout, KH, KW, stride, pad_lo, pad_hi, ep, stream, nullptr);
}

IDIFF_API const char *idiff_conv2d_route(const void *x, const void *wt, const void *out, int B, int H, int W, int Cin, int Cout, int KH,
                                         int KW, int stride, int pad_lo, int pad_hi, const idiff_epilogue *ep) {
  IgemmPlan c = {};
  if (conv_front((const float *)x, (const float *)wt, (float *)const_cast<void *>(out), B, H, W, Cin, Cout, KH, KW, stride, pad_lo, pad_hi, ep,
                 nullptr, &c))
    return nullptr;
  return c.family < 0 ? "none" : igemm_plan_name(c);
}


IDIFF_API int idiff_gemm_colstats_split(int M, int N, int K, int64_t lda, int64_t ldb, int rows_per_sample) {
  if (M <= 0 || N <= 0 || K <= 0 || rows_per_sample <= 0 || M % rows_per_sample || idiff::option(idiff::OPT_NO_COLSTATS)) return 0;
  if (pipe_serves_linear(M, N, K, lda, ldb) != PIPE_YES) return 0;
// ... 14 lines not shown
```

id-diff_amd/csrc/runtime.hip:

```cpp
#include "common.h"
#include <stdlib.h>
#include <string.h>
#include <limits.h>

namespace idiff {
static thread_local char g_err[512] = "";
void set_error(const char *fmt, ...) {
  va_list ap;
  va_start(ap, fmt);
  vsnprintf(g_err, sizeof(g_err), fmt, ap);
  va_end(ap);
}

namespace {
const char *const kOptionNames[OPT_COUNT] = {"IDIFF_NO_WINOGRAD", "IDIFF_NO_COLSTATS", "IDIFF_NO_PIPE", "IDIFF_SCALAR_EPILOGUE",
                                             "IDIFF_DBUF_ONLY", "IDIFF_TRIDIAG_ONESTAGE", "IDIFF_UFD_ROWS", "IDIFF_CHASE_WAVEFRONT",
                                             "IDIFF_WINO_NGROUP", "IDIFF_GRAM_SMALL_TILES", "IDIFF_CHASE_SPIN_LIMIT",
                                             "IDIFF_FAKE_CU_COUNT", "IDIFF_SBR_SYNC", "IDIFF_SBR_FULL", "IDIFF_NO_SPLIT", "IDIFF_WINO_SPLIT", "IDIFF_SBR_LOOKAHEAD",
                                             "IDIFF_NO_WINO43", "IDIFF_NO_WINO43H", "IDIFF_NO_PAIRS", "IDIFF_PAIRS_MIN_TILES", "IDIFF_NO_FUSED_ATTN", "IDIFF_NO_WINO1D", "IDIFF_NO_FUSED_GN", "IDIFF_NO_FUSED_GN_LOAD", "IDIFF_NO_FUSED_GN_LOAD_2SRC", "IDIFF_NO_FUSED_GN_FIR"};
struct OptionTable {
  int v[OPT_COUNT];
  OptionTable() {
    for (int i = 0; i < OPT_COUNT; ++i) { const char *e = getenv(kOptionNames[i]); v[i] = (e && *e) ? atoi(e) : 0; }
  }
};
OptionTable g_options;
constexpr int kUnset = INT_MIN;
struct ThreadOptions {
  int v[OPT_COUNT];
  ThreadOptions() { for (int i = 0; i < OPT_COUNT; ++i) v[i] = kUnset; }
};
thread_local ThreadOptions t_options;
}

int option_value(Option o) {
  const int t = t_options.v[o];
  return t != kUnset ? t : __atomic_load_n(&g_options.v[o], __ATOMIC_RELAXED);
}
bool option(Option o) { return option_value(o) != 0; }

int set_dynamic_lds_once(AttrGuard &g, const void *const *fns, int n_fns, int bytes, const char *what) {
  int dev = 0;
  hipError_t e = hipGetDevice(&dev);
  if (e != hipSuccess) { set_error("%s: hipGetDevice: %s", what, hipGetErrorString(e)); return (int)e; }
  const unsigned long long bit = 1ull << (dev & 63);
  if (__atomic_load_n(&g.done_mask, __ATOMIC_ACQUIRE) & bit) return 0;
  for (int i = 0; i < n_fns; ++i) {
    e = hipFuncSetAttribute(fns[i], hipFuncAttributeMaxDynamicSharedMemorySize, bytes);
    if (e != hipSuccess) { set_error("%s: hipFuncSetAttribute: %s", what, hipGetErrorString(e)); return (int)e; }
  }
  __atomic_fetch_or(&g.done_mask, bit, __ATOMIC_RELEASE);
  return 0;
}
}

#ifndef IDIFF_SOURCE_STAMP
#define IDIFF_SOURCE_STAMP "unstamped"
#endif
IDIFF_API int idiff_abi_version(void) { return IDIFF_ABI_VERSION; }
IDIFF_API const char *idiff_source_stamp(void) { return IDIFF_SOURCE_STAMP; }
#ifndef IDIFF_VARIANT_FLAGS
#define IDIFF_VARIANT_FLAGS ""
#endif
IDIFF_API const char *idiff_variant_flags(void) { return IDIFF_VARIANT_FLAGS; }
IDIFF_API const char *idiff_last_error(void) { return idiff::g_err; }

IDIFF_API int idiff_set_option(const char *name, int value) {
  using namespace idiff;
  if (!name) return -1;
  for (int i = 0; i < OPT_COUNT; ++i)
    if (strcmp(name, kOptionNames[i]) == 0) return __atomic_exchange_n(&g_options.v[i], value, __ATOMIC_RELAXED);
  return -1;
}

IDIFF_API int idiff_set_thread_option(const char *name, int value, int set) {
  using namespace idiff;
  if (!name) return -1;
  for (int i = 0; i < OPT_COUNT; ++i)
    if (strcmp(name, kOptionNames[i]) == 0) { t_options.v[i] = set ? value : kUnset; return 0; }
  return -1;
}
```

id-diff_amd/csrc/upfirdn2d.hip:

```cpp
#include "common.h"
#include <stdlib.h>
#include <algorithm>

namespace {

struct UfdParams {
  int major, in_h, in_w, minor, kh, kw;
  int up_x, up_y, down_x, down_y, pad_x0, pad_y0;
  int out_h, out_w;
};

__device__ __forceinline__ int floor_div(int a, int b) {
  int q = a / b;
  return (a % b != 0 && a < 0) ? q - 1 : q;
}
__device__ __forceinline__ int ceil_div_s(int a, int b) { return -floor_div(-a, b); }

constexpr int kMaxTaps = 64;

struct GroupPlan { int ppb, grid, ngroups; };
template <typename LdsBytes, typename Admissible>
GroupPlan plan_plane_groups(int major, int ppb_max, LdsBytes lds_bytes_of, Admissible admissible) {
  if (lds_bytes_of(1) > 64 * 1024) return {0, 0, 0};
  GroupPlan best = {1, major, major};
// ... 462 lines not shown
        for (int u = 0; u < 2; ++u)
#pragma unroll
          for (int v = 0; v < 2; ++v) {
            const float wt = w[(a + 2 * u) * 4 + (b + 2 * v)];
            const float4 sv = in[a + u][b + v];
            acc.x += sv.x * wt; acc.y += sv.y * wt; acc.z += sv.z * wt; acc.w += sv.w * wt;
          }
        op[((int64_t)a * p.out_w + 2 * j + b) * cv] = acc;
      }
  }
}

template <int ACT>
__device__ __forceinline__ float4 gn_act4(const float4 s, const float4 c01, const float4 c23) {
  return make_float4(idiff::act_apply(fmaf(c01.x, s.x, c01.y), ACT), idiff::act_apply(fmaf(c01.z, s.y, c01.w), ACT),
                     idiff::act_apply(fmaf(c23.x, s.z, c23.y), ACT), idiff::act_apply(fmaf(c23.z, s.w, c23.w), ACT));
}

template <int ACT>
__global__ void __launch_bounds__(256)
upfirdn2d_nhwc_down2_block_gn(const float *__restrict__ x, const float *__restrict__ k, const float *__restrict__ coef,
                              float *__restrict__ out, UfdParams p, int cv, int col_step) {
  __shared__ float taps[16];
  if (threadIdx.x < 16) {
    const int ky = threadIdx.x >> 2, kx = threadIdx.x & 3;
    taps[threadIdx.x] = k[(3 - ky) * 4 + (3 - kx)];
  }
  __syncthreads();
  const int bid = xcd_contiguous(blockIdx.x, gridDim.x);
  const int brows = (p.out_h + 1) >> 1;
  const int plane = bid / brows, Y = bid - plane * brows;
  const int c4 = threadIdx.x % cv, col0 = threadIdx.x / cv;
  if (col0 >= col_step) return;
  float w[16];
#pragma unroll
  for (int t = 0; t < 16; ++t) w[t] = __builtin_bit_cast(float, __builtin_amdgcn_readfirstlane(__builtin_bit_cast(int, taps[t])));
  const float4 *cp = reinterpret_cast<const float4 *>(coef) + ((int64_t)plane * cv + c4) * 2;
  const float4 c01 = cp[0], c23 = cp[1];
  const int by = 4 * Y - p.pad_y0;
  const bool row1 = 2 * Y + 1 < p.out_h;
  const float4 *xp = reinterpret_cast<const float4 *>(x) + (int64_t)plane * p.in_h * p.in_w * cv + c4;
  float4 *op = reinterpret_cast<float4 *>(out) + ((int64_t)plane * p.out_h + 2 * Y) * p.out_w * cv + c4;
  const float4 zero = make_float4(0.f, 0.f, 0.f, 0.f);
  for (int X = col0; 2 * X < p.out_w; X += col_step) {
    const int bx = 4 * X - p.pad_x0;
    float4 acc[2][2] = {{zero, zero}, {zero, zero}};
#pragma unroll
    for (int rr = 0; rr < 6; ++rr) {
      const int iy = by + rr;
      const bool vy = (unsigned)iy < (unsigned)p.in_h;
      const float4 *row = xp + (int64_t)(vy ? iy : 0) * p.in_w * cv;
      float4 s[6];
#pragma unroll
      for (int cc = 0; cc < 6; ++cc) {
        const int ix = bx + cc;
        const bool ok = vy && (unsigned)ix < (unsigned)p.in_w;
        const float4 v = gn_act4<ACT>(row[(int64_t)(ok ? ix : 0) * cv], c01, c23);
        s[cc] = ok ? v : zero;
      }
#pragma unroll
      for (int a = 0; a < 2; ++a) {
        const int ky = rr - 2 * a;
        if (ky < 0 || ky > 3) continue;
#pragma unroll
        for (int b = 0; b < 2; ++b)
#pragma unroll
          for (int t = 0; t < 4; ++t) {
            const float wt = w[ky * 4 + t];
            const float4 sv = s[t + 2 * b];
            acc[a][b].x += sv.x * wt; acc[a][b].y += sv.y * wt; acc[a][b].z += sv.z * wt; acc[a][b].w += sv.w * wt;
          }
      }
    }
    const bool col1 = 2 * X + 1 < p.out_w;
    op[(int64_t)(2 * X) * cv] = acc[0][0];
    if (col1) op[(int64_t)(2 * X + 1) * cv] = acc[0][1];
    if (row1) {
      op[((int64_t)p.out_w + 2 * X) * cv] = acc[1][0];
      if (col1) op[((int64_t)p.out_w + 2 * X + 1) * cv] = acc[1][1];
    }
  }
}

template <int ACT>
__global__ void __launch_bounds__(256)
upfirdn2d_nhwc_up2_block_gn(const float *__restrict__ x, const float *__restrict__ k, const float *__restrict__ coef,
                            float *__restrict__ out, UfdParams p, int cv, int col_step) {
  __shared__ float taps[16];
  if (threadIdx.x < 16) {
    const int ky = threadIdx.x >> 2, kx = threadIdx.x & 3;
    taps[threadIdx.x] = k[(3 - ky) * 4 + (3 - kx)];
  }
  __syncthreads();
  const int bid = xcd_contiguous(blockIdx.x, gridDim.x);
  const int plane = bid / p.in_h, i = bid - plane * p.in_h;
  const int c4 = threadIdx.x % cv, col0 = threadIdx.x / cv;
  if (col0 >= col_step) return;
  float w[16];
#pragma unroll
  for (int t = 0; t < 16; ++t) w[t] = __builtin_bit_cast(float, __builtin_amdgcn_readfirstlane(__builtin_bit_cast(int, taps[t])));
  const float4 *cp = reinterpret_cast<const float4 *>(coef) + ((int64_t)plane * cv + c4) * 2;
  const float4 c01 = cp[0], c23 = cp[1];
  const float4 *xp = reinterpret_cast<const float4 *>(x) + (int64_t)plane * p.in_h * p.in_w * cv + c4;
  float4 *op = reinterpret_cast<float4 *>(out) + ((int64_t)plane * p.out_h + 2 * i) * p.out_w * cv + c4;
  const float4 zero = make_float4(0.f, 0.f, 0.f, 0.f);
  const int per = (p.in_w + col_step - 1) / col_step;
  const int j0 = col0 * per, j1 = min(j0 + per, p.in_w);
  if (j0 >= j1) return;
  const float4 *row[3];
  bool vy[3];
#pragma unroll
  for (int r = 0; r < 3; ++r) {
    const int iy = i - 1 + r;
    vy[r] = (unsigned)iy < (unsigned)p.in_h;
    row[r] = xp + (int64_t)(vy[r] ? iy : 0) * p.in_w * cv;
  }
  auto raw = [&](int r, int ix) { return row[r][(int64_t)((unsigned)ix < (unsigned)p.in_w ? ix : 0) * cv]; };
  auto normed = [&](int r, int ix, const float4 v) { return (vy[r] && (unsigned)ix < (unsigned)p.in_w) ? gn_act4<ACT>(v, c01, c23) : zero; };
  float4 in[3][3];
#pragma unroll
  for (int r = 0; r < 3; ++r) {
    in[r][1] = normed(r, j0 - 1, raw(r, j0 - 1));
    in[r][2] = normed(r, j0, raw(r, j0));
  }
  for (int j = j0; j < j1; ++j) {
    float4 nxt[3];
#pragma unroll
    for (int r = 0; r < 3; ++r) {
      in[r][0] = in[r][1]; in[r][1] = in[r][2];
      nxt[r] = raw(r, j + 1);
    }
#pragma unroll
    for (int r = 0; r < 3; ++r) in[r][2] = normed(r, j + 1, nxt[r]);
#pragma unroll
    for (int a = 0; a < 2; ++a)
#pragma unroll
      for (int b = 0; b < 2; ++b) {
        float4 acc = zero;
#pragma unroll
        for (int u = 0; u < 2; ++u)
#pragma unroll
          for (int v = 0; v < 2; ++v) {
            const float wt = w[(a + 2 * u) * 4 + (b + 2 * v)];
            const float4 sv = in[a + u][b + v];
            acc.x += sv.x * wt; acc.y += sv.y * wt; acc.z += sv.z * wt; acc.w += sv.w * wt;
          }
        op[((int64_t)a * p.out_w + 2 * j + b) * cv] = acc;
      }
  }
}

__global__ void __launch_bounds__(256)
upfirdn2d_generic(const float *__restrict__ x, const float *__restrict__ k, float *__restrict__ out, UfdParams p,
                  int64_t total) {
  for (int64_t v = (int64_t)blockIdx.x * blockDim.x + threadIdx.x; v < total; v += (int64_t)gridDim.x * blockDim.x) {
    int c = (int)(v % p.minor);
    int64_t pix = v / p.minor;
    int ox = (int)(pix % p.out_w);
    int64_t t = pix / p.out_w;
    int oy = (int)(t % p.out_h);
    int64_t plane = t / p.out_h;
    const int by = oy * p.down_y - p.pad_y0, bx = ox * p.down_x - p.pad_x0;
    const int iy_lo = max(ceil_div_s(by, p.up_y), 0), iy_hi = min(floor_div(by + p.kh - 1, p.up_y), p.in_h - 1);
    const int ix_lo = max(ceil_div_s(bx, p.up_x), 0), ix_hi = min(floor_div(bx + p.kw - 1, p.up_x), p.in_w - 1);
    float acc = 0.f;
    for (int iy = iy_lo; iy <= iy_hi; ++iy) {
      const int ky = iy * p.up_y - by;
      for (int ix = ix_lo; ix <= ix_hi; ++ix) {
        const int kx = ix * p.up_x - bx;
        acc += x[((plane * p.in_h + iy) * p.in_w + ix) * p.minor + c] * k[(p.kh - 1 - ky) * p.kw + (p.kw - 1 - kx)];
      }
    }
    out[v] = acc;
  }
}

template <typename T, typename ACC>
__global__ void __launch_bounds__(256)
upfirdn2d_generic_t(const T *__restrict__ x, const T *__restrict__ k, T *__restrict__ out, UfdParams p, int64_t total) {
  for (int64_t v = (int64_t)blockIdx.x * blockDim.x + threadIdx.x; v < total; v += (int64_t)gridDim.x * blockDim.x) {
    int c = (int)(v % p.minor);
    int64_t pix = v / p.minor;
    int ox = (int)(pix % p.out_w);
    int64_t t = pix / p.out_w;
    int oy = (int)(t % p.out_h);
    int64_t plane = t / p.out_h;
    const int by = oy * p.down_y - p.pad_y0, bx = ox * p.down_x - p.pad_x0;
    const int iy_lo = max(ceil_div_s(by, p.up_y), 0), iy_hi = min(floor_div(by + p.kh - 1, p.up_y), p.in_h - 1);
    const int ix_lo = max(ceil_div_s(bx, p.up_x), 0), ix_hi = min(floor_div(bx + p.kw - 1, p.up_x), p.in_w - 1);
    ACC acc = (ACC)0;
    for (int iy = iy_lo; iy <= iy_hi; ++iy) {
      const int ky = iy * p.up_y - by;
      for (int ix = ix_lo; ix <= ix_hi; ++ix) {
        const int kx = ix * p.up_x - bx;
        acc += (ACC)x[((plane * p.in_h + iy) * p.in_w + ix) * p.minor + c] * (ACC)k[(p.kh - 1 - ky) * p.kw + (p.kw - 1 - kx)];
      }
    }
    out[v] = (T)acc;
  }
}

int ufd_geometry(int major, int in_h, int in_w, int minor, int kh, int kw, int up_x, int up_y, int down_x, int down_y, int pad_x0,
                 int pad_x1, int pad_y0, int pad_y1, UfdParams &p) {
  using namespace idiff;
  if (major < 0 || in_h <= 0 || in_w <= 0 || minor <= 0 || kh <= 0 || kw <= 0)
    return fail("upfirdn2d: bad shape major=%d in=%dx%d minor=%d k=%dx%d", major, in_h, in_w, minor, kh, kw);
  if (up_x < 1 || up_y < 1 || down_x < 1 || down_y < 1) return fail("upfirdn2d: up/down factors must be >= 1");
  p.major = major; p.in_h = in_h; p.in_w = in_w; p.minor = minor; p.kh = kh; p.kw = kw;
  p.up_x = up_x; p.up_y = up_y; p.down_x = down_x; p.down_y = down_y; p.pad_x0 = pad_x0; p.pad_y0 = pad_y0;
  const int span_h = in_h * up_y + pad_y0 + pad_y1 - kh, span_w = in_w * up_x + pad_x0 + pad_x1 - kw;
  if (span_h < 0 || span_w < 0) return fail("upfirdn2d: kernel larger than padded input");
  p.out_h = span_h / down_y + 1;
  p.out_w = span_w / down_x + 1;
  return 0;
}

template <typename T, typename ACC>
int ufd_launch_t(const void *x, const void *k, void *out, int major, int in_h, int in_w, int minor, int kh, int kw, int up_x, int up_y,
                 int down_x, int down_y, int pad_x0, int pad_x1, int pad_y0, int pad_y1, void *stream, const char *what) {
  UfdParams p;
  if (major != 0 && (!x || !k || !out)) return idiff::fail("upfirdn2d: null pointer");
  if (int rc = ufd_geometry(major, in_h, in_w, minor, kh, kw, up_x, up_y, down_x, down_y, pad_x0, pad_x1, pad_y0, pad_y1, p))
    return rc;
  if (major == 0) return 0;
  const int64_t total = (int64_t)major * p.out_h * p.out_w * minor;
  hipLaunchKernelGGL((upfirdn2d_generic_t<T, ACC>), dim3(idiff::streaming_grid(total, 256)), dim3(256), 0, (hipStream_t)stream,
                     (const T *)x, (const T *)k, (T *)out, p, total);
  return idiff::launch_status(what);
}

enum UfdRoute {
  UFD_NONE,
  UFD_PLANES_FIR4, UFD_PLANES_ROWSLIDE, UFD_PLANES_DOWN2, UFD_PLANES_WHOLE0, UFD_PLANES_WHOLE1, UFD_PLANES_WHOLE_ANY,
  UFD_PLANES_LDS, UFD_NHWC_UP2_BLOCK, UFD_NHWC_ROWS0, UFD_NHWC_ROWS1, UFD_NHWC_ROWS_ANY, UFD_NHWC_VEC4, UFD_GENERIC,
};
const char *const kUfdRouteNames[] = {"none", "planes_fir4", "planes_rowslide", "planes_down2", "planes_whole<0>", "planes_whole<1>",
                                      "planes_whole<-1>", "planes_lds", "nhwc_up2_block", "nhwc_rows<0>", "nhwc_rows<1>",
                                      "nhwc_rows<-1>", "nhwc_vec4", "generic"};

struct UfdPlan {
  UfdRoute route;
  dim3 grid;
  size_t lds;
  int ppb, ngroups, rows, pitch;
  int tx_log2;
  int toh, tow, tih, tiw, tiles_x;
  int cv, col_step;
  int64_t total;
};

int ufd_choose(const void *x, const void *out, int major, int in_h, int in_w, int minor, int kh, int kw, int up_x, int up_y,
               int down_x, int down_y, int pad_x0, int pad_x1, int pad_y0, int pad_y1, UfdParams &p, UfdPlan &c) {
  using namespace idiff;
  if (major != 0 && (!x || !out)) return fail("upfirdn2d: null pointer");
  if (int rc = ufd_geometry(major, in_h, in_w, minor, kh, kw, up_x, up_y, down_x, down_y, pad_x0, pad_x1, pad_y0, pad_y1, p))
    return rc;
  c = UfdPlan{};
  c.route = UFD_NONE;
  if (major == 0) return 0;
  const int64_t total = (int64_t)major * p.out_h * p.out_w * minor;

  if (minor == 1 && up_x == 1 && up_y == 1 && down_x == 1 && down_y == 1 && kh <= 4 && kw <= 4 && pad_x0 >= 0 && pad_y0 >= 0 &&
      pad_x0 <= 4 && pad_y0 <= 4 && in_w % 4 == 0 && (int64_t)in_h * in_w <= 4096 && ((uintptr_t)x & 15) == 0 && !option(OPT_UFD_ROWS)) {
    const int rows = max(in_h + pad_y0, p.out_h + 3), pitch = (max(in_w + pad_x0, 4 * ((p.out_w + 3) / 4) + 4) + 3) & ~3;
    const int fsz = rows * pitch;
    auto lds_of = [&](int ppb) { return (size_t)ppb * fsz * sizeof(float); };
    const GroupPlan g = plan_plane_groups(major, std::min(major, 64), lds_of, [](int) { return true; });
    if (g.ppb > 0) {
      c.route = UFD_PLANES_FIR4; c.grid = dim3(g.grid); c.lds = lds_of(g.ppb); c.ppb = g.ppb; c.ngroups = g.ngroups;
      c.rows = rows; c.pitch = pitch;
      return 0;
    }
  }
  if (minor == 1 && up_x == 1 && up_y == 1 && down_x == 1 && down_y == 1 && kh <= 4 && kw <= 4 && p.out_h <= 128 &&
      (int64_t)in_h * in_w <= 4096) {
    const int lpsz = in_h * (in_w + 1), osz = p.out_h * p.out_w;
    auto lds_of = [&](int ppb) { return (16 + (size_t)ppb * (lpsz + osz)) * sizeof(float); };
    const GroupPlan g = plan_plane_groups(major, max(1, 256 / p.out_h), lds_of, [](int) { return true; });
    if (g.ppb > 0) {
      c.route = UFD_PLANES_ROWSLIDE; c.grid = dim3(g.grid); c.lds = lds_of(g.ppb); c.ppb = g.ppb; c.ngroups = g.ngroups;
      return 0;
    }
  }
  if (minor == 1 && up_x == 1 && up_y == 1 && down_x == 2 && down_y == 2 && kh <= 4 && kw <= 4 && pad_x0 >= 0 && pad_y0 >= 0 &&
      pad_x0 <= 4 && pad_y0 <= 4 && p.out_h % 2 == 0 && p.out_w % 2 == 0 && in_w % 4 == 0 && (int64_t)in_h * in_w <= 4096 &&
      (((uintptr_t)x | (uintptr_t)out) & 15) == 0 && !option(OPT_UFD_ROWS)) {
    const int rows = max(in_h + pad_y0, 2 * p.out_h + 2), pitch = (max(in_w + pad_x0, 2 * p.out_w + 2) + 3) & ~3;
    const int fsz = rows * pitch, nb = (p.out_h / 2) * (p.out_w / 2);
    auto lds_of = [&](int ppb) { return (size_t)ppb * fsz * sizeof(float); };
    auto full_rounds = [&](int ppb) {
      if (nb >= 256 || 256 % nb != 0) return true;
      const int unit = 256 / nb;
      return ppb % unit == 0 || (major < unit && ppb == major);
    };
    const GroupPlan g = plan_plane_groups(major, std::min(major, 64), lds_of, full_rounds);
    if (g.ppb > 0) {
      c.route = UFD_PLANES_DOWN2; c.grid = dim3(g.grid); c.lds = lds_of(g.ppb); c.ppb = g.ppb; c.ngroups = g.ngroups;
      c.rows = rows; c.pitch = pitch;
      return 0;
    }
  }
  if (minor == 1 && kh * kw <= kMaxTaps && (int64_t)in_h * in_w <= 8192 && (int64_t)p.out_h * p.out_w <= 16384) {
    const int psz = in_h * in_w, osz = p.out_h * p.out_w;
    int ppb = max(1, min((32 * 1024 / 4) / psz, 4096 / max(osz, 1)));
    ppb = max(1, min(ppb, max(1, major / 1024)));
    int tx_log2 = 0;
    while ((1 << tx_log2) < min(p.out_w, 64)) ++tx_log2;
    const int uplog = (up_x == up_y && kh <= 4 && kw <= 4) ? (up_x == 1 ? 0 : up_x == 2 ? 1 : -1) : -1;
    c.route = uplog == 0 ? UFD_PLANES_WHOLE0 : uplog == 1 ? UFD_PLANES_WHOLE1 : UFD_PLANES_WHOLE_ANY;
    c.grid = dim3(ceil_div(major, ppb)); c.lds = (kMaxTaps + (size_t)ppb * psz) * sizeof(float); c.ppb = ppb; c.tx_log2 = tx_log2;
    return 0;
  }
  if (minor == 1 && kh * kw <= kMaxTaps) {
    const int tow = min(p.out_w, 64), toh = min(p.out_h, 32);
    const int tih = ((toh - 1) * down_y + kh - 1) / up_y + 2;
    const int tiw = ((tow - 1) * down_x + kw - 1) / up_x + 2;
    const int tile_elems = toh * tow;
    int ppb = max(1, 2048 / tile_elems);
    const int max_ppb_lds = max(1, (int)((48 * 1024 / sizeof(float) - kMaxTaps) / (tih * (tiw + 1))));
    ppb = min(min(ppb, max_ppb_lds), major);
    const size_t lds_bytes = (kMaxTaps + (size_t)ppb * tih * (tiw + 1)) * sizeof(float);
    if (lds_bytes <= 64 * 1024) {
      const int tiles_x = ceil_div(p.out_w, tow), tiles_y = ceil_div(p.out_h, toh);
      const dim3 grid(ceil_div(major, ppb), tiles_x * tiles_y);
      if (grid.y <= 65535) {
        c.route = UFD_PLANES_LDS; c.grid = grid; c.lds = lds_bytes; c.ppb = ppb;
        c.toh = toh; c.tow = tow; c.tih = tih; c.tiw = tiw; c.tiles_x = tiles_x;
        return 0;
      }
    }
  }
  constexpr int64_t kMaxRowGroups = 0xffffffffll / 256;
  if (minor % 4 == 0 && minor <= 1024 && kh * kw <= kMaxTaps && ((uintptr_t)x % 16 == 0) && ((uintptr_t)out % 16 == 0) &&
      (int64_t)major * p.out_h <= kMaxRowGroups) {
    c.cv = minor / 4; c.col_step = 256 / c.cv;
    const int gx = (int64_t)major * p.out_h >= 2048 ? 1 : max(1, min(ceil_div(p.out_w, c.col_step), 8));
    if (up_x == 2 && up_y == 2 && down_x == 1 && down_y == 1 && kh == 4 && kw == 4 && pad_x0 == 2 && pad_y0 == 2 &&
        p.out_h == 2 * in_h && p.out_w == 2 * in_w && (int64_t)major * in_h <= kMaxRowGroups && !option(OPT_UFD_ROWS)) {
      c.route = UFD_NHWC_UP2_BLOCK; c.grid = dim3(major * in_h);
      return 0;
    }
    const int uplog = (up_x == up_y && kh <= 4 && kw <= 4) ? (up_x == 1 ? 0 : up_x == 2 ? 1 : -1) : -1;
    c.route = uplog == 0 ? UFD_NHWC_ROWS0 : uplog == 1 ? UFD_NHWC_ROWS1 : UFD_NHWC_ROWS_ANY;
    c.grid = dim3(major * p.out_h, gx);
    return 0;
  }
  if (minor % 4 == 0 && kh * kw <= kMaxTaps && ((uintptr_t)x % 16 == 0) && ((uintptr_t)out % 16 == 0)) {
    c.route = UFD_NHWC_VEC4; c.total = total / 4; c.grid = dim3(streaming_grid(c.total, 256));
    return 0;
  }
  c.route = UFD_GENERIC; c.total = total; c.grid = dim3(streaming_grid(total, 256));
  return 0;
}

}

IDIFF_API int idiff_upfirdn2d_f16(const void *x, const void *k, void *out, int major, int in_h, int in_w, int minor, int kh, int kw,
                                  int up_x, int up_y, int down_x, int down_y, int pad_x0, int pad_x1, int pad_y0, int pad_y1,
                                  void *stream) {
  return ufd_launch_t<_Float16, float>(x, k, out, major, in_h, in_w, minor, kh, kw, up_x, up_y, down_x, down_y, pad_x0, pad_x1, pad_y0,
                                       pad_y1, stream, "upfirdn2d_f16");
}

IDIFF_API int idiff_upfirdn2d_f64(const double *x, const double *k, double *out, int major, int in_h, int in_w, int minor, int kh,
                                  int kw, int up_x, int up_y, int down_x, int down_y, int pad_x0, int pad_x1, int pad_y0, int pad_y1,
                                  void *stream) {
  return ufd_launch_t<double, double>(x, k, out, major, in_h, in_w, minor, kh, kw, up_x, up_y, down_x, down_y, pad_x0, pad_x1, pad_y0,
                                      pad_y1, stream, "upfirdn2d_f64");
}

IDIFF_API int idiff_upfirdn2d_f32(const float *x, const float *k, float *out, int major, int in_h, int in_w,
                                  int minor, int kh, int kw, int up_x, int up_y, int down_x, int down_y,
                                  int pad_x0, int pad_x1, int pad_y0, int pad_y1, void *stream) {
  using namespace idiff;
  if (major != 0 && !k) return fail("upfirdn2d: null pointer");
  UfdParams p;
  UfdPlan c;
  if (int rc = ufd_choose(x, out, major, in_h, in_w, minor, kh, kw, up_x, up_y, down_x, down_y, pad_x0, pad_x1, pad_y0, pad_y1, p, c))
    return rc;
  hipStream_t st = (hipStream_t)stream;
  const dim3 blk(256);
  switch (c.route) {
    case UFD_NONE: return 0;
    case UFD_PLANES_FIR4:
      hipLaunchKernelGGL(upfirdn2d_planes_fir4, c.grid, blk, c.lds, st, x, k, out, p, c.ppb, c.rows, c.pitch, c.ngroups);
      return launch_status("upfirdn2d_planes_fir4");
    case UFD_PLANES_ROWSLIDE:
      hipLaunchKernelGGL(upfirdn2d_planes_rowslide, c.grid, blk, c.lds, st, x, k, out, p, c.ppb, c.ngroups);
      return launch_status("upfirdn2d_planes_rowslide");
    case UFD_PLANES_DOWN2:
      hipLaunchKernelGGL(upfirdn2d_planes_down2, c.grid, blk, c.lds, st, x, k, out, p, c.ppb, c.rows, c.pitch, c.ngroups);
      return launch_status("upfirdn2d_planes_down2");
    case UFD_PLANES_WHOLE0:
      hipLaunchKernelGGL(upfirdn2d_planes_whole<0>, c.grid, blk, c.lds, st, x, k, out, p, c.ppb, c.tx_log2);
      return launch_status("upfirdn2d_planes_whole");
    case UFD_PLANES_WHOLE1:
      hipLaunchKernelGGL(upfirdn2d_planes_whole<1>, c.grid, blk, c.lds, st, x, k, out, p, c.ppb, c.tx_log2);
      return launch_status("upfirdn2d_planes_whole");
    case UFD_PLANES_WHOLE_ANY:
      hipLaunchKernelGGL(upfirdn2d_planes_whole<-1>, c.grid, blk, c.lds, st, x, k, out, p, c.ppb, c.tx_log2);
      return launch_status("upfirdn2d_planes_whole");
    case UFD_PLANES_LDS:
      hipLaunchKernelGGL(upfirdn2d_planes_lds, c.grid, blk, c.lds, st, x, k, out, p, c.toh, c.tow, c.tih, c.tiw, c.ppb, c.tiles_x);
      return launch_status("upfirdn2d_planes_lds");
    case UFD_NHWC_UP2_BLOCK:
      hipLaunchKernelGGL(upfirdn2d_nhwc_up2_block, c.grid, blk, 0, st, x, k, out, p, c.cv, c.col_step);
      return launch_status("upfirdn2d_nhwc_up2_block");
    case UFD_NHWC_ROWS0:
      hipLaunchKernelGGL(upfirdn2d_nhwc_rows<0>, c.grid, blk, 0, st, x, k, out, p, c.cv, c.col_step);
      return launch_status("upfirdn2d_nhwc_rows");
    case UFD_NHWC_ROWS1:
      hipLaunchKernelGGL(upfirdn2d_nhwc_rows<1>, c.grid, blk, 0, st, x, k, out, p, c.cv, c.col_step);
      return launch_status("upfirdn2d_nhwc_rows");
    case UFD_NHWC_ROWS_ANY:
      hipLaunchKernelGGL(upfirdn2d_nhwc_rows<-1>, c.grid, blk, 0, st, x, k, out, p, c.cv, c.col_step);
      return launch_status("upfirdn2d_nhwc_rows");
    case UFD_NHWC_VEC4:
      hipLaunchKernelGGL(upfirdn2d_nhwc_vec4, c.grid, blk, 0, st, x, k, out, p, c.total);
      return launch_status("upfirdn2d_nhwc_vec4");
    case UFD_GENERIC:
      hipLaunchKernelGGL(upfirdn2d_generic, c.grid, blk, 0, st, x, k, out, p, c.total);
      return launch_status("upfirdn2d_generic");
  }
  return fail("upfirdn2d: no route");
}

IDIFF_API const char *idiff_upfirdn2d_route(const void *x, const void *out, int major, int in_h, int in_w, int minor, int kh, int kw,
                                            int up_x, int up_y, int down_x, int down_y, int pad_x0, int pad_x1, int pad_y0,
                                            int pad_y1) {
  UfdParams p;
  UfdPlan c;
  if (ufd_choose(x, out, major, in_h, in_w, minor, kh, kw, up_x, up_y, down_x, down_y, pad_x0, pad_x1, pad_y0, pad_y1, p, c)) return nullptr;
  return kUfdRouteNames[c.route];
}

namespace {
int ufd_gn_choose(const void *x, const void *coef, int act, const void *out, int major, int in_h, int in_w, int minor, int kh, int kw,
                  int up_x, int up_y, int down_x, int down_y, int pad_x0, int pad_x1, int pad_y0, int pad_y1, UfdParams &p, UfdPlan &c) {
  using namespace idiff;
  if (act != IDIFF_ACT_NONE && act != IDIFF_ACT_SILU) return fail("upfirdn2d_gn: activation code %d (none or SiLU are served)", act);
  if (major != 0 && !coef) return fail("upfirdn2d_gn: null coefficients");
  if ((uintptr_t)coef % 16) return fail("upfirdn2d_gn: coefficients not 16-byte aligned");
  if (int rc = ufd_choose(x, out, major, in_h, in_w, minor, kh, kw, up_x, up_y, down_x, down_y, pad_x0, pad_x1, pad_y0, pad_y1, p, c))
    return rc;
  const bool down2 = c.route == UFD_NHWC_ROWS0 && down_x == 2 && down_y == 2 && kh == 4 && kw == 4;
  if (c.route != UFD_NONE && c.route != UFD_NHWC_UP2_BLOCK && !down2)
    return fail("upfirdn2d_gn: served where upfirdn2d takes nhwc_up2_block (up 2, 4x4 taps) or nhwc_rows<0> with down 2 and 4x4 taps "
                "(minor %% 4 == 0), this geometry takes %s with down %dx%d and %dx%d taps", kUfdRouteNames[c.route], down_x, down_y, kh, kw);
  if (down2) c.grid = dim3(major * ((p.out_h + 1) / 2));
  return 0;
}
}

IDIFF_API int idiff_upfirdn2d_gn_f32(const float *x, const float *k, const float *coef, int act, float *out, int major, int in_h,
                                     int in_w, int minor, int kh, int kw, int up_x, int up_y, int down_x, int down_y, int pad_x0,
                                     int pad_x1, int pad_y0, int pad_y1, void *stream) {
  using namespace idiff;
  if (major != 0 && !k) return fail("upfirdn2d_gn: null pointer");
  UfdParams p;
  UfdPlan c;
  if (int rc = ufd_gn_choose(x, coef, act, out, major, in_h, in_w, minor, kh, kw, up_x, up_y, down_x, down_y, pad_x0, pad_x1, pad_y0,
                             pad_y1, p, c))
    return rc;
  hipStream_t st = (hipStream_t)stream;
  const dim3 blk(256);
  const bool silu = act == IDIFF_ACT_SILU;
  switch (c.route) {
    case UFD_NONE: return 0;
    case UFD_NHWC_UP2_BLOCK:
      if (silu) hipLaunchKernelGGL(upfirdn2d_nhwc_up2_block_gn<IDIFF_ACT_SILU>, c.grid, blk, 0, st, x, k, coef, out, p, c.cv, c.col_step);
      else hipLaunchKernelGGL(upfirdn2d_nhwc_up2_block_gn<IDIFF_ACT_NONE>, c.grid, blk, 0, st, x, k, coef, out, p, c.cv, c.col_step);
      return launch_status("upfirdn2d_nhwc_up2_block_gn");
    case UFD_NHWC_ROWS0:
      if (silu) hipLaunchKernelGGL(upfirdn2d_nhwc_down2_block_gn<IDIFF_ACT_SILU>, c.grid, blk, 0, st, x, k, coef, out, p, c.cv, c.col_step);
      else hipLaunchKernelGGL(upfirdn2d_nhwc_down2_block_gn<IDIFF_ACT_NONE>, c.grid, blk, 0, st, x, k, coef, out, p, c.cv, c.col_step);
      return launch_status("upfirdn2d_nhwc_down2_block_gn");
    default: break;
  }
  return fail("upfirdn2d_gn: no route");
}

IDIFF_API int idiff_upfirdn2d_gn_ok(const void *x, const void *coef, int act, const void *out, int major, int in_h, int in_w, int minor,
                                    int kh, int kw, int up_x, int up_y, int down_x, int down_y, int pad_x0, int pad_x1, int pad_y0,
                                    int pad_y1) {
  if (idiff::option(idiff::OPT_NO_FUSED_GN_FIR)) return 0;
  UfdParams p;
  UfdPlan c;
  if (ufd_gn_choose(x, coef, act, out, major, in_h, in_w, minor, kh, kw, up_x, up_y, down_x, down_y, pad_x0, pad_x1, pad_y0, pad_y1, p, c))
// ... 5 lines not shown
```

id-diff_amd/models/beatgans.py:

```python
import torch
import torch.nn as nn

from .. import _lib
from . import utils
from .nhwc import NhwcExecutor, _T, _pad4


def _normalization(ch):
    return nn.GroupNorm(min(32, ch), ch)


def _zero(module):
    for p in module.parameters():
        p.detach().zero_()
    return module


class Resample(nn.Module):

    def __init__(self, channels, use_conv, up, out_channels=None):
        super().__init__()
        self.up, self.use_conv = up, use_conv
        out_channels = out_channels or channels
        if use_conv and up:
# ... 77 lines not shown
        heads_up = m.num_heads if m.num_heads_upsample == -1 else m.num_heads_upsample
        zero = m.resnet_use_zero_module

        def res(ch, out=None, **kw):
            return ResBlock(ch, E, m.dropout, out_channels=out, use_zero_module=zero, **kw)

        def attn(ch, heads):
            return AttentionBlock(ch, heads, m.num_head_channels, m.use_new_attention_order)

        ch = input_ch = int(mults[0] * self.mc)
        self.input_blocks = nn.ModuleList([Block(nn.Conv2d(m.in_channels, ch, 3, padding=1))])
        chans = [[] for _ in mults]
        chans[0].append(ch)
        self.input_num_blocks = [0] * len(mults)
        self.input_num_blocks[0] = 1
        self.output_num_blocks = [0] * len(mults)
        resolution = m.image_size
        for level, mult in enumerate(in_mults):
            for _ in range(m.num_input_res_blocks or m.num_res_blocks):
                layers = [res(ch, int(mult * self.mc))]
                ch = int(mult * self.mc)
                if resolution in m.attention_resolutions:
                    layers.append(attn(ch, m.num_heads))
                self.input_blocks.append(Block(*layers))
                chans[level].append(ch)
                self.input_num_blocks[level] += 1
            if level != len(mults) - 1:
                resolution //= 2
                self.input_blocks.append(Block(res(ch, ch, down=True) if m.resblock_updown
                                               else Resample(ch, m.conv_resample, False, ch)))
                chans[level + 1].append(ch)
                self.input_num_blocks[level + 1] += 1
        self.middle_block = Block(res(ch), attn(ch, m.num_heads), res(ch))
        self.output_blocks = nn.ModuleList([])
        for level, mult in list(enumerate(mults))[::-1]:
            for i in range(m.num_res_blocks + 1):
                ich = chans[level].pop() if chans[level] else 0
                layers = [res(ch + ich, int(self.mc * mult), has_lateral=ich > 0)]
                ch = int(self.mc * mult)
                if resolution in m.attention_resolutions:
                    layers.append(attn(ch, heads_up))
                if level and i == m.num_res_blocks:
                    resolution *= 2
                    layers.append(res(ch, ch, up=True) if m.resblock_updown else Resample(ch, m.conv_resample, True, ch))
                self.output_blocks.append(Block(*layers))
                self.output_num_blocks[level] += 1
        out_conv = nn.Conv2d(input_ch, m.out_channels, 3, padding=1)
        self.out = nn.Sequential(_normalization(ch), nn.SiLU(), _zero(out_conv) if zero else out_conv)

    def _pack(self):
        pk = {"conv": {}, "lin": {}, "emb_off": {}}
        ws, bs, off = [], [], 0
        for mod in self.modules():
            if isinstance(mod, ResBlock):
                pk["emb_off"][id(mod)] = off
                lin = mod.emb_layers[1]
                ws.append(lin.weight.detach().float())
                bs.append(lin.bias.detach().float())
                off += 2 * mod.out_channels
        pk["emb_w"] = torch.cat(ws, 0).contiguous()
        pk["emb_b"] = torch.cat(bs, 0).contiguous()
        return pk

    def _cw(self, pk, conv, split=None):
        key = (id(conv), split)
        if key not in pk["conv"]:
            pk["conv"][key] = (self._pack_conv(conv, split), conv.bias.detach().float().contiguous())
        return pk["conv"][key]

    def _resblock(self, mod, x, emb_all, pk, lateral=None):
        x2 = lateral if mod.has_lateral else None
        assert x.C + (x2.C if x2 is not None else 0) == mod.channels
        h = self._gn_act(x, mod.in_layers[0], "silu", x2)
        if mod.up or mod.down:
            assert x2 is None
            h, x = self._box(h, mod.up), self._box(x, mod.up)
        w0, b0 = self._cw(pk, mod.in_layers[2])
        h = self._conv(h, w0, b0, stats=True, normed=True)
        off = pk["emb_off"][id(mod)]
        h = self._gn_act(h, mod.out_layers[0], "silu", mod=emb_all[:, off:off + 2 * mod.out_channels])
        if isinstance(mod.skip_connection, nn.Identity):
            sc = x if x2 is None else self._cat(x, x2)
        else:
            split = x.C if x2 is not None else None
            ws, bsk = self._cw(pk, mod.skip_connection, split)
            if x2 is None:
                sc = self._pointwise(x, ws.view(ws.shape[0], -1), bsk)
            else:
                part = self._pointwise(x, ws[0].view(ws[0].shape[0], -1), bsk)
                sc = self._pointwise(x2, ws[1].view(ws[1].shape[0], -1), None, residual=part.buf)
        w1, b1 = self._cw(pk, mod.out_layers[3])
        return self._conv(h, w1, b1, residual=sc.buf, stats=True, normed=True)

    def _attn(self, mod, x, pk):
        C = x.C
        n = self._gn_act(x, mod.norm, None)
        key = (id(mod), "qkv")
        if key not in pk["lin"]:
            w = mod.qkv.weight.detach().float().view(3 * C, C)
            b = mod.qkv.bias.detach().float()
            pk["lin"][key] = (*pack_qkv_heads(w, b, mod.num_heads, mod.use_new_attention_order),
                              mod.proj_out.weight.detach().float().view(C, C).contiguous(),
                              mod.proj_out.bias.detach().float().contiguous())
        return self._attention(pk, x, n, mod.norm, *pk["lin"][key], pk["lin"], (id(mod), "attn_scale"), heads=mod.num_heads)

    def _resample(self, mod, x, pk):
        if mod.up:
            x = self._box(x, True)
            if mod.use_conv:
                w, b = self._cw(pk, mod.conv)
                x = self._conv(x, w, b)
            return x
        if mod.use_conv:
            w, b = self._cw(pk, mod.op)
            return self._conv(x, w, b, stride=2, pad=1)
        return self._box(x, False)

    def _run_block(self, block, x, emb_all, pk, lateral=None):
        for layer in block:
            if isinstance(layer, ResBlock):
                x = self._resblock(layer, x, emb_all, pk, lateral)
            elif isinstance(layer, AttentionBlock):
                x = self._attn(layer, x, pk)
            elif isinstance(layer, Resample):
                x = self._resample(layer, x, pk)
            elif isinstance(layer, nn.Conv2d):
                w, b = self._cw(pk, layer)
                x = self._conv(x, w, b)
            else:
                raise TypeError(type(layer))
        return x

    forward_accepts_out = True

    def forward(self, x, t, out_rowscale=None, out=None):
        x, t = self._check_inputs(x, t)
        if x.ndim != 4 or x.shape[1] != self.channels:
            raise RuntimeError(f"BeatGANsUNetModel: expected [B, {self.channels}, H, W], got {tuple(x.shape)}")
        pk = self.packed()
        B, C, H, W = x.shape
        dev = x.device
        temb = torch.empty(B, self.temb_ch, device=dev, dtype=torch.float32)
        _lib.positional_embed(t, temb, B, self.temb_ch, 10000.0, mode=1)
        l0, l2 = self.time_embed[0], self.time_embed[2]
        e1 = _lib.gemm(temb, l0.weight.detach(), epilogue=_lib.make_epilogue(bias=l0.bias.detach(), act="silu"))
        e2 = _lib.gemm(e1, l2.weight.detach(), epilogue=_lib.make_epilogue(bias=l2.bias.detach(), act="silu"))
        emb_all = _lib.gemm(e2, pk["emb_w"], epilogue=_lib.make_epilogue(bias=pk["emb_b"]))
        cp = _pad4(C)
        h = _T(torch.empty(B, H * W, cp, device=dev, dtype=torch.float32), H, W, cp)
        _lib.nchw_to_nhwc(x, h.buf, B, C, H * W, cp)
        hs = [[] for _ in self.input_num_blocks]
        k = 0
        for i, nb in enumerate(self.input_num_blocks):
            for _ in range(nb):
                h = self._run_block(self.input_blocks[k], h, emb_all, pk)
                hs[i].append(h)
                k += 1
        h = self._run_block(self.middle_block, h, emb_all, pk)
        k = 0
        for i, nb in enumerate(self.output_num_blocks):
            for _ in range(nb):
                lateral = hs[-i - 1].pop() if hs[-i - 1] else None
                h = self._run_block(self.output_blocks[k], h, emb_all, pk, lateral)
                k += 1
        n = self._gn_act(h, self.out[0], "silu")
        w, b = self._cw(pk, self.out[2])
        h = self._conv(n, w, b, normed=True)
        out = self._out_buffer(out, B, C, H, W, dev)
        _lib.nhwc_to_nchw(h.buf, out, B, C, H * W, h.C, out_rowscale)
        return out
# ... 1 lines not shown
```

id-diff_amd/models/ncsnpp.py:

```python
import math
import os

import numpy as np
import torch
import torch.nn as nn

from .. import _lib
from . import utils
from .nhwc import NhwcExecutor, _T, _pad4

_INV_SQRT2 = float(1.0 / np.sqrt(2.0))


def _fan_avg_uniform(shape, scale=1.):
    scale = 1e-10 if scale == 0 else scale
    rf = np.prod(shape) / shape[1] / shape[0]
    variance = scale / ((shape[1] * rf + shape[0] * rf) / 2)
    return (torch.rand(*shape) * 2. - 1.) * np.sqrt(3 * variance)


def _conv(cin, cout, k, init_scale=1., stride=1, padding=None):
    conv = nn.Conv2d(cin, cout, k, stride=stride, padding=(k // 2 if padding is None else padding))
    conv.weight.data = _fan_avg_uniform(conv.weight.shape, init_scale)
    nn.init.zeros_(conv.bias)
# ... 226 lines not shown
        pk["fir_down"] = torch.tensor(k, device=dev)
        pk["fir_up"] = torch.tensor(k * 4.0, device=dev)
        pk["fir_len"] = int(k.shape[0])
        pk["fir_gain"] = {"down": float(np.abs(k).sum()), "pre_conv": float(np.abs(k).sum()),
                          "up": float(max(np.abs(4.0 * k[py::2, px::2]).sum() for py in (0, 1) for px in (0, 1)))}
        dense_w, dense_b, off = [], [], 0
        for i, mod in enumerate(M):
            if isinstance(mod, (ResnetBlockBigGANpp, ResnetBlockDDPMpp)):
                pk["dense_off"][i] = off
                dense_w.append(mod.Dense_0.weight.detach().float())
                dense_b.append(mod.Dense_0.bias.detach().float())
                off += mod.out_ch
        pk["dense_w"] = torch.cat(dense_w, 0).contiguous()
        pk["dense_b"] = torch.cat(dense_b, 0).contiguous()
        pk["dense_total"] = off
        return pk

    def _conv_w(self, pk, key, conv, cin_split=None):
        if key not in pk["conv"]:
            pk["conv"][key] = (self._pack_conv(conv, cin_split), conv.bias.detach().float().contiguous())
        return pk["conv"][key]

    def _nin_w(self, pk, key, nin, cin_split=None):
        if key not in pk["nin"]:
            pk["nin"][key] = (self._pack_nin(nin, cin_split), nin.b.detach().float().contiguous())
        return pk["nin"][key]

    def _fir(self, x, pk, mode, gn=None, act=None):
        B = x.buf.shape[0]
        n = pk["fir_len"]
        if mode == "up":
            p = n - 2
            k, up, down, p0, p1 = pk["fir_up"], 2, 1, (p + 1) // 2 + 1, p // 2
        elif mode == "down":
            p = n - 2
            k, up, down, p0, p1 = pk["fir_down"], 1, 2, (p + 1) // 2, p // 2
        else:
            p = (n - 2) + 2
            k, up, down, p0, p1 = pk["fir_down"], 1, 1, (p + 1) // 2, p // 2
        OH = _lib.upfirdn2d_out_size(x.H, up, down, p0, p1, n)
        OW = _lib.upfirdn2d_out_size(x.W, up, down, p0, p1, n)
        if gn is not None:
            if x.stats is None or x.pending is not None or _lib.ACT[act] not in (0, 1) or x.C % gn.num_groups or x.C % 4:
                return None
            coef = torch.empty(B * x.C * 2, device=x.buf.device, dtype=torch.float32)
            y = self._new(B, OH, OW, x.C, x.buf)
            if not _lib.upfirdn2d_gn_ok(x.buf, coef, act, y.buf, B, x.H, x.W, x.C, n, n, up, up, down, down, p0, p1, p0, p1):
                return None
            _lib.groupnorm_reader_coef(x.stats[0], x.stats[1], x.C, B, x.H * x.W, gn.num_groups, gn.eps, gn.weight.detach(),
                                       gn.bias.detach(), coef)
            _lib.upfirdn2d_gn(x.buf, k, coef, act, y.buf, B, x.H, x.W, x.C, up, up, down, down, p0, p1, p0, p1)
            y.norm = (gn, (x.C // gn.num_groups) * x.H * x.W, pk["fir_gain"][mode], False)
            return y
        y = self._new(B, OH, OW, x.C, x.buf)
        _lib.upfirdn2d_raw(x.buf, k, y.buf, B, x.H, x.W, x.C, up, up, down, down, p0, p1, p0, p1)
        if x.norm is not None:
            y.norm = (x.norm[0], x.norm[1], x.norm[2] * pk["fir_gain"][mode], x.norm[3])
        return y

    def _resblock(self, idx, x, temb_all, pk, x2=None):
        mod = self.all_modules[idx]
        rs = _INV_SQRT2 if self.skip_rescale else 1.0
        c_in = x.C + (x2.C if x2 is not None else 0)
        assert c_in == mod.in_ch, (c_in, mod.in_ch)
        early_shortcut = False
        if mod.up or mod.down:
            assert x2 is None
            h = self._fir(x, pk, "up" if mod.up else "down", gn=mod.GroupNorm_0, act=self.act_name) if self.fir else None
            if h is None:
                h = self._gn_act(x, mod.GroupNorm_0, self.act_name)
                h = self._fir(h, pk, "up" if mod.up else "down") if self.fir else self._box(h, mod.up)
            resample = (lambda t: self._fir(t, pk, "up" if mod.up else "down")) if self.fir else (lambda t: self._box(t, mod.up))
            early_shortcut = SHORTCUT_BEFORE_UPSAMPLE and mod.up and (hasattr(mod, "Conv_2") or hasattr(mod, "NIN_0"))
            if not early_shortcut:
                x = resample(x)
        else:
            h = self._gn_act(x, mod.GroupNorm_0, self.act_name, x2, conv_cout=mod.out_ch)
        w0, b0 = self._conv_w(pk, (idx, 0), mod.Conv_0)
        off = pk["dense_off"][idx]
        h = self._conv_gn_act(h, w0, b0, mod.GroupNorm_1, self.act_name, rowbias=temb_all[:, off:off + mod.out_ch], normed=True,
                              next_cout=mod.out_ch)
        if hasattr(mod, "Conv_2") or hasattr(mod, "NIN_0"):
            fused = x2 is not None and x.C == x2.C and x.C % 32 == 0
            split = x.C if (x2 is not None and not fused) else None
            if hasattr(mod, "Conv_2"):
                ws, bs = self._conv_w(pk, (idx, 2), mod.Conv_2, split)
                ws = [w.view(w.shape[0], -1) for w in ws] if split is not None else ws.view(ws.shape[0], -1)
            else:
                ws, bs = self._nin_w(pk, (idx, "nin"), mod.NIN_0, split)
            if early_shortcut:
                sc = resample(self._pointwise(x, ws, None))
            elif x2 is None:
                sc = self._pointwise(x, ws, bs)
            elif fused:
                sc = self._new(x.buf.shape[0], x.H, x.W, ws.shape[0], x.buf)
                _lib.gemm_2src(x.buf.view(-1, x.C), x2.buf.view(-1, x2.C), ws, sc.buf.view(-1, ws.shape[0]),
                               epilogue=_lib.make_epilogue(bias=bs))
            else:
                part = self._pointwise(x, ws[0], bs)
                sc = self._pointwise(x2, ws[1], None, residual=part.buf)
        else:
            assert x2 is None
            sc = x
        w1, b1 = self._conv_w(pk, (idx, 1), mod.Conv_1)
        if early_shortcut:
            if (idx, "1+shortcut") not in pk["conv"]:
                pk["conv"][(idx, "1+shortcut")] = (w1, (b1 + bs).contiguous())
            b1 = pk["conv"][(idx, "1+shortcut")][1]
        return self._conv(h, w1, b1, residual=sc.buf, out_scale=rs, stats=True, normed=True)

    def _attn(self, idx, x, pk):
        mod = self.all_modules[idx]
        n = self._gn_act(x, mod.GroupNorm_0, None)
        if (idx, "qk") not in pk["nin"]:
            wq, bq = self._nin_w(pk, (idx, 0), mod.NIN_0)
            wk, bk = self._nin_w(pk, (idx, 1), mod.NIN_1)
            pk["nin"][(idx, "qk")] = (torch.cat([wq, wk], 0).contiguous(), torch.cat([bq, bk], 0).contiguous())
        return self._attention(pk, x, n, mod.GroupNorm_0, *pk["nin"][(idx, "qk")], *self._nin_w(pk, (idx, 2), mod.NIN_2),
                               *self._nin_w(pk, (idx, 3), mod.NIN_3), pk["nin"], (idx, "attn_scale"),
                               out_scale=_INV_SQRT2 if self.skip_rescale else 1.0)

    def _downsample(self, idx, x, pk, **ep):
        mod = self.all_modules[idx] if isinstance(idx, int) else idx
        if mod.fir:
            if not mod.with_conv:
                return self._fir(x, pk, "down")
            key = (id(mod), "firconv")
            if key not in pk["conv"]:
                pk["conv"][key] = (self._pack_conv(mod.Conv2d_0), mod.Conv2d_0.bias.detach().float().contiguous())
            w, b = pk["conv"][key]
            return self._conv(self._fir(x, pk, "pre_conv"), w, b, stride=2, pad=0, **ep)
        if mod.with_conv:
            w, b = self._conv_w(pk, (id(mod), "conv"), mod.Conv_0)
            return self._conv(x, w, b, stride=2, pad=0, pad_hi=1, **ep)
        return self._box(x, False)

    forward_accepts_out = True

    def forward(self, x, time_cond, out_rowscale=None, out=None):
        x, time_cond = self._check_inputs(x, time_cond)
        if x.ndim != 4 or x.shape[1] != self.channels:
            raise RuntimeError(f"ncsnpp: expected [B, {self.channels}, H, W], got {tuple(x.shape)}")
        pk = self.packed()
        M = self.all_modules
        B, C, H, W = x.shape
        dev = x.device
        cp = _pad4(C)
        rs = _INV_SQRT2 if self.skip_rescale else 1.0
        temb = temb_all = h = pyr_in = pyr = None
        hs = []
        for step in self._plan:
            op = step[0]
            if op == "fourier":
                half = self.nf
                temb = torch.empty(B, 2 * half, device=dev, dtype=torch.float32)
                _lib.fourier_embed(time_cond, M[step[1]].W.detach(), temb, B, half)
            elif op == "positional":
                temb = torch.empty(B, self.nf, device=dev, dtype=torch.float32)
                _lib.positional_embed(time_cond, temb, B, self.nf)
            elif op == "temb_mlp":
                l0, l1 = M[step[1]], M[step[2]]
                t1 = _lib.gemm(temb, l0.weight.detach(), epilogue=_lib.make_epilogue(bias=l0.bias.detach(), act=self.act_name))
                t2 = _lib.gemm(t1, l1.weight.detach(), epilogue=_lib.make_epilogue(bias=l1.bias.detach(), act=self.act_name))
                temb_all = _lib.gemm(t2, pk["dense_w"], epilogue=_lib.make_epilogue(bias=pk["dense_b"]))
            elif op == "stem":
                xin = _T(torch.empty(B, H * W, cp, device=dev, dtype=torch.float32), H, W, cp)
                if self.centered:
                    _lib.nchw_to_nhwc(x, xin.buf, B, C, H * W, cp)
                else:
                    _lib.nchw_to_nhwc(x, xin.buf, B, C, H * W, cp, 2.0, -1.0)
                pyr_in = xin
                w, b = self._conv_w(pk, (step[1], "stem"), M[step[1]])
                hs = [self._conv(xin, w, b, stats=True)]
            elif op == "res_push":
                h = self._resblock(step[1], hs[-1], temb_all, pk)
                if step[2] is not None:
                    h = self._attn(step[2], h, pk)
                hs.append(h)
            elif op == "down":
                _, i_down, is_res, mode, i_pyr = step
# ... 59 lines not shown
```

include/idiff_hip.h:

```cpp
#ifndef IDIFF_HIP_H
#define IDIFF_HIP_H

#include <stdint.h>

#ifdef __cplusplus
extern "C" {
#endif

#define IDIFF_EINVAL 1001
#define IDIFF_ABI_VERSION 1

int idiff_abi_version(void);
const char *idiff_last_error(void);
const char *idiff_source_stamp(void);
const char *idiff_variant_flags(void);

int idiff_set_option(const char *name, int value);

int idiff_set_thread_option(const char *name, int value, int set);


int idiff_upfirdn2d_f32(const float *x, const float *k, float *out, int major, int in_h, int in_w, int minor,
                        int kh, int kw, int up_x, int up_y, int down_x, int down_y, int pad_x0, int pad_x1,
                        int pad_y0, int pad_y1, void *stream);

const char *idiff_upfirdn2d_route(const void *x, const void *out, int major, int in_h, int in_w, int minor, int kh, int kw,
                                  int up_x, int up_y, int down_x, int down_y, int pad_x0, int pad_x1, int pad_y0, int pad_y1);

int idiff_upfirdn2d_gn_f32(const float *x, const float *k, const float *coef, int act, float *out, int major, int in_h, int in_w,
                           int minor, int kh, int kw, int up_x, int up_y, int down_x, int down_y, int pad_x0, int pad_x1, int pad_y0,
                           int pad_y1, void *stream);
int idiff_upfirdn2d_gn_ok(const void *x, const void *coef, int act, const void *out, int major, int in_h, int in_w, int minor, int kh,
                          int kw, int up_x, int up_y, int down_x, int down_y, int pad_x0, int pad_x1, int pad_y0, int pad_y1);

int idiff_fused_bias_act_f32(const float *x, const float *b, const float *ref, float *out, int64_t n,
                             int step_b, int size_b, int act, int grad, float alpha, float scale, void *stream);

int idiff_upfirdn2d_f16(const void *x, const void *k, void *out, int major, int in_h, int in_w, int minor, int kh, int kw,
                        int up_x, int up_y, int down_x, int down_y, int pad_x0, int pad_x1, int pad_y0, int pad_y1, void *stream);
int idiff_upfirdn2d_f64(const double *x, const double *k, double *out, int major, int in_h, int in_w, int minor, int kh, int kw,
                        int up_x, int up_y, int down_x, int down_y, int pad_x0, int pad_x1, int pad_y0, int pad_y1, void *stream);
int idiff_fused_bias_act_f16(const void *x, const void *b, const void *ref, void *out, int64_t n, int step_b, int size_b,
                             int act, int grad, float alpha, float scale, void *stream);
int idiff_fused_bias_act_f64(const double *x, const double *b, const double *ref, double *out, int64_t n, int step_b,
                             int size_b, int act, int grad, float alpha, float scale, void *stream);


#define IDIFF_ACT_NONE 0
#define IDIFF_ACT_SILU 1
#define IDIFF_ACT_ELU 2
#define IDIFF_ACT_RELU 3
#define IDIFF_ACT_LRELU 4

typedef struct idiff_epilogue {
  const float *bias;
  const float *rowbias;
  int64_t ld_rowbias;
  int rows_per_group;
  int act;
  const float *residual;
  int64_t ld_residual;
  float out_scale;
  const float *rowscale;
  double *colstats;
} idiff_epilogue;

int idiff_gemm_f32(const float *A, int64_t lda, int64_t strideA, const float *Bt, int64_t ldb, int64_t strideB,
                   float *C, int64_t ldc, int64_t strideC, int M, int N, int K, int batch,
                   const idiff_epilogue *ep, void *stream);

int idiff_gemm_pairs_ok(int M, int N, int K, int batch);
int idiff_gemm_pairs_scale_f32(const float *w, int64_t ldw, int rows, int K, float *w_scale, void *stream);
int idiff_gemm_pairs_f32(const float *A, int64_t lda, int64_t strideA, const float *Bt, int64_t ldb, int64_t strideB,
                         const float *w_scale, int weight_is_a, const float *act_scale, float *C, int64_t ldc, int64_t strideC,
                         int M, int N, int K, int batch, const idiff_epilogue *ep, void *stream);

int idiff_pairs_act_scale_f32(const double *ws1, int nsplit1, int C1, const double *ws2, int nsplit2, int C2, int B, int HW, float *out,
                              void *stream);
int idiff_gemm_pairs_2src_f32(const float *A1, const float *A2, int64_t lda, int K1, const float *act_scale, const float *Bt, int64_t ldb,
                              const float *w_scale, float *C, int64_t ldc, int M, int N, int K, const idiff_epilogue *ep, void *stream);

int idiff_gemm_2src_f32(const float *A1, const float *A2, int64_t lda, int K1, const float *Bt, int64_t ldb, float *C,
                        int64_t ldc, int M, int N, int K, const idiff_epilogue *ep, void *stream);

int idiff_conv2d_nhwc_f32(const float *x, const float *wt, float *out, int B, int H, int W, int Cin, int Cout,
                          int KH, int KW, int stride, int pad_lo, int pad_hi, const idiff_epilogue *ep, void *stream);

const char *idiff_gemm_route(const void *A, int64_t lda, int64_t strideA, const void *Bt, int64_t ldb, int64_t strideB, const void *C,
                             int64_t ldc, int64_t strideC, int M, int N, int K, int batch, const idiff_epilogue *ep, int pairs);
const char *idiff_conv2d_route(const void *x, const void *wt, const void *out, int B, int H, int W, int Cin, int Cout, int KH, int KW,
                               int stride, int pad_lo, int pad_hi, const idiff_epilogue *ep);

int idiff_gemm_colstats_split(int M, int N, int K, int64_t lda, int64_t ldb, int rows_per_sample);
int idiff_conv2d_colstats_split(int B, int H, int W, int Cin, int Cout, int KH, int KW, int stride, int pad_lo,
                                int pad_hi);

int idiff_conv2d_winograd_ok(int B, int H, int W, int Cin, int Cout);
int64_t idiff_winograd_weight_floats(int Cin, int Cout);
int idiff_winograd_pack_f32(const float *wt, float *u, int Cin, int Cout, void *stream);
int idiff_conv2d_winograd_f32(const float *x, const float *u, float *out, int B, int H, int W, int Cin, int Cout,
                              const idiff_epilogue *ep, void *stream);
int idiff_conv2d_winograd_colstats_split(int B, int H, int W, int Cin, int Cout);
int idiff_conv2d_winograd43_ok(int B, int H, int W, int Cin, int Cout);
int idiff_conv2d_winograd43_colstats_split(int B, int H, int W, int Cin, int Cout);
int64_t idiff_winograd43_weight_floats(int Cin, int Cout);
int idiff_winograd43_pack_f32(const float *wt, float *u, int Cin, int Cout, void *stream);
int idiff_conv2d_winograd43_f32(const float *x, const float *u, float *out, int B, int H, int W, int Cin, int Cout,
                                const idiff_epilogue *ep, void *stream);
int idiff_conv2d_winograd43h_ok(int B, int H, int W, int Cin, int Cout);
int64_t idiff_winograd43h_weight_floats(int Cin, int Cout);
int idiff_winograd43h_pack_f32(const float *wt, float *u, int Cin, int Cout, void *stream);
int idiff_conv2d_winograd43h_f32(const float *x, const float *u, float *out, int B, int H, int W, int Cin, int Cout,
                                 const idiff_epilogue *ep, void *stream);

int idiff_conv2d_wino1d_ok(int B, int H, int W, int Cin, int Cout);
int idiff_conv2d_wino1d_colstats_split(int B, int H, int W, int Cin, int Cout);
int64_t idiff_wino1d_weight_floats(int Cin, int Cout);
int idiff_wino1d_pack_f32(const float *wt, float *u, int Cin, int Cout, void *stream);
int idiff_conv2d_wino1d_f32(const float *x, const float *u, float *out, int B, int H, int W, int Cin, int Cout,
                            const idiff_epilogue *ep, void *stream);
int idiff_conv2d_wino1d_gn_ok(int B, int H, int W, int Cin, int Cout, int groups);
int idiff_conv2d_wino1d_gn_f32(const float *x, const float *u, float *out, int B, int H, int W, int Cin, int Cout,
                               const idiff_epilogue *ep, int groups, const float *gamma, const float *beta, float eps, int act,
                               void *stream);
int idiff_conv2d_wino1d_normload_ok(int B, int H, int W, int Cin, int Cout);
int idiff_conv2d_wino1d_normload_f32(const float *x, const float *u, float *out, int B, int H, int W, int Cin, int Cout,
                                     const idiff_epilogue *ep, const float *coef, int act, void *stream);
int idiff_conv2d_wino1d_normload_2src_ok(int B, int H, int W, int C1, int C2, int Cout);
int idiff_conv2d_wino1d_normload_2src_f32(const float *x1, int C1, const float *x2, int C2, const float *u, float *out, int B, int H, int W,
                                          int Cout, const idiff_epilogue *ep, const float *coef, int act, void *stream);

int idiff_conv2d_winograd_split_ok(int B, int H, int W, int Cin, int Cout);
int64_t idiff_winograd_split_weight_floats(int Cin, int Cout);
int idiff_winograd_pack_split_f32(const float *wt, float *u, int Cin, int Cout, void *stream);
int idiff_conv2d_winograd_split_f32(const float *x, const float *u, float *out, int B, int H, int W, int Cin, int Cout,
                                    const idiff_epilogue *ep, void *stream);


int idiff_groupnorm_nsplit(int B, int HW, int C);
int idiff_groupnorm_stats_f32(const float *x, int C, const float *x2, int C2, int B, int HW, int G, float eps,
                              double *workspace, float *stats, void *stream);
int idiff_groupnorm_finalize_f32(const double *ws1, int nsplit1, int C1, const double *ws2, int nsplit2, int C2, int B,
                                 int HW, int G, float eps, float *stats, void *stream);
int idiff_groupnorm_apply_f32(const float *x, int C, const float *x2, int C2, int B, int HW, int G,
                              const float *stats, const float *gamma, const float *beta, const float *mod,
                              int64_t ld_mod, int act, float *y, void *stream);
int idiff_groupnorm_apply_colstats_f32(const float *x, int C, const float *x2, int C2, int B, int HW, int G,
                                       const double *ws1, int nsplit1, const double *ws2, int nsplit2, float eps,
                                       const float *gamma, const float *beta, const float *mod, int64_t ld_mod,
                                       int act, float *y, void *stream);
const char *idiff_groupnorm_apply_route(const void *x, int C, const void *x2, int C2, int B, int HW, int G, const void *stats,
                                        const void *gamma, const void *beta, const void *y);
const char *idiff_groupnorm_apply_colstats_route(const void *x, int C, const void *x2, int C2, int B, int HW, int G,
                                                 const double *ws1, int nsplit1, const double *ws2, int nsplit2,
                                                 const void *gamma, const void *beta, const void *y);
int idiff_groupnorm_coef_f32(const double *ws1, int nsplit1, int C1, const double *ws2, int nsplit2, int C2, int B, int HW, int G,
                             float eps, const float *gamma, const float *beta, float *coef, void *stream);

int idiff_softmax_rows_f32(const float *x, float *y, int64_t rows, int cols, float scale, void *stream);
const char *idiff_softmax_rows_route(const void *x, const void *y, int64_t rows, int cols, float scale);

int idiff_attention256_ok(int B, int tokens, int C);
int idiff_attention256_f32(const float *qk, int64_t ld_qk, const float *vt, const float *bias_v, const float *s_qk, const float *s_v,
                           float *out, int B, int tokens, int C, float scale, void *stream);

int idiff_attention_heads_ok(int B, int tokens, int H, int D);
// ... 163 lines not shown
```

Before: 19090.

## Fuse unequal-width two-source skip GEMMs and route up2 FIR through sliding kernel

Adds a two-source GEMM variant whose second operand has its own row pitch. The ncsnpp and beatgans residual-block shortcuts on concatenated inputs of different channel counts now run as one fused GEMM instead of two pointwise GEMMs plus a residual add, which removes one launch and one extra read-write of the output. Separately, the plain up2 upfirdn path is rerouted through the GN-fused block kernel with normalization compiled out when rows are long enough. This adds more kernel template instantiations and per-row pitch arithmetic in the A loads.

```diff
diff --git a/id-diff_amd/_lib.py b/id-diff_amd/_lib.py
--- a/id-diff_amd/_lib.py
+++ b/id-diff_amd/_lib.py
@@ -44,6 +44,9 @@
     "idiff_gemm_f32": (c_i, [c_p, c_i64, c_i64, c_p, c_i64, c_i64, c_p, c_i64, c_i64, c_i, c_i, c_i, c_i,
                              ctypes.POINTER(Epilogue), c_p]),
     "idiff_gemm_2src_f32": (c_i, [c_p, c_p, c_i64, c_i, c_p, c_i64, c_p, c_i64, c_i, c_i, c_i, ctypes.POINTER(Epilogue), c_p]),
+    "idiff_gemm_2src_ld_f32": (c_i, [c_p, c_i64, c_i, c_p, c_i64, c_i, c_p, c_i64, c_p, c_i64, c_i, c_i, ctypes.POINTER(Epilogue), c_p]),
+    "idiff_gemm_2src_ld_ok": (c_i, [c_i, c_i, c_i, c_i, c_i64, c_i64, c_i64]),
+    "idiff_gemm_2src_ld_route": (ctypes.c_char_p, [c_p, c_i64, c_i, c_p, c_i64, c_i, c_p, c_i64, c_p, c_i64, c_i, c_i, ctypes.POINTER(Epilogue)]),
     "idiff_conv2d_nhwc_f32": (c_i, [c_p, c_p, c_p] + [c_i] * 10 + [ctypes.POINTER(Epilogue), c_p]),
     "idiff_gemm_route": (ctypes.c_char_p, [c_p, c_i64, c_i64, c_p, c_i64, c_i64, c_p, c_i64, c_i64, c_i, c_i, c_i, c_i,
                                            ctypes.POINTER(Epilogue), c_i]),
@@ -510,6 +513,30 @@
     return out
 
 
+def gemm_2src_ld(a1, a2, bt, out, epilogue=None):
+    _dev(a1, "a1", contiguous=False); _dev(a2, "a2", contiguous=False); _dev(bt, "bt"); _dev(out, "out")
+    M, K1 = a1.shape
+    K2 = a2.shape[1]
+    if a2.shape[0] != M or a1.stride(1) != 1 or a2.stride(1) != 1 or bt.shape[1] != K1 + K2 or out.shape[0] != M or out.shape[1] != bt.shape[0]:
+        raise RuntimeError(f"gemm_2src_ld: shapes {tuple(a1.shape)} | {tuple(a2.shape)} x {tuple(bt.shape)}^T -> {tuple(out.shape)}")
+    ep = _ep_ref(epilogue, "gemm_2src_ld")
+    _check(lib().idiff_gemm_2src_ld_f32(a1.data_ptr(), a1.stride(0), K1, a2.data_ptr(), a2.stride(0), K2, bt.data_ptr(), bt.stride(0),
+                                        out.data_ptr(), out.stride(0), M, bt.shape[0], ep, _stream()), "idiff_gemm_2src_ld_f32")
+    return out
+
+
+def gemm_2src_ld_ok(M, N, K1, K2, lda1=None, lda2=None, ldb=None):
+    return bool(lib().idiff_gemm_2src_ld_ok(M, N, K1, K2, K1 if lda1 is None else lda1, K2 if lda2 is None else lda2,
+                                            K1 + K2 if ldb is None else ldb))
+
+
+def gemm_2src_ld_route(a1, a2, bt, out, epilogue=None):
+    ep = _ep_ref(epilogue, "gemm_2src_ld")
+    r = lib().idiff_gemm_2src_ld_route(a1.data_ptr(), a1.stride(0), a1.shape[1], a2.data_ptr(), a2.stride(0), a2.shape[1], bt.data_ptr(),
+                                       bt.stride(0), out.data_ptr(), out.stride(0), a1.shape[0], bt.shape[0], ep)
+    return r.decode() if r is not None else None
+
+
 def conv2d_nhwc(x, wt, out, B, H, W, Cin, Cout, KH, KW, stride, pad, epilogue=None, pad_hi=None):
     ep = _ep_ref(epilogue, "conv2d_nhwc")
     _check(lib().idiff_conv2d_nhwc_f32(x.data_ptr(), wt.data_ptr(), out.data_ptr(), B, H, W, Cin, Cout, KH, KW, stride,
diff --git a/id-diff_amd/csrc/common.h b/id-diff_amd/csrc/common.h
--- a/id-diff_amd/csrc/common.h
+++ b/id-diff_amd/csrc/common.h
@@ -33,7 +33,7 @@
 
 enum Option { OPT_NO_WINOGRAD, OPT_NO_COLSTATS, OPT_NO_PIPE, OPT_SCALAR_EPILOGUE, OPT_DBUF_ONLY, OPT_TRIDIAG_ONESTAGE,
               OPT_UFD_ROWS, OPT_CHASE_WAVEFRONT, OPT_WINO_NGROUP, OPT_GRAM_SMALL_TILES, OPT_CHASE_SPIN_LIMIT, OPT_FAKE_CU_COUNT,
-              OPT_SBR_SYNC, OPT_SBR_FULL, OPT_NO_SPLIT, OPT_WINO_SPLIT, OPT_SBR_LOOKAHEAD, OPT_NO_WINO43, OPT_NO_WINO43H, OPT_NO_PAIRS, OPT_PAIRS_MIN_TILES, OPT_NO_FUSED_ATTN, OPT_NO_WINO1D, OPT_NO_FUSED_GN, OPT_NO_FUSED_GN_LOAD, OPT_NO_FUSED_GN_LOAD_2SRC, OPT_NO_FUSED_GN_FIR, OPT_COUNT };
+              OPT_SBR_SYNC, OPT_SBR_FULL, OPT_NO_SPLIT, OPT_WINO_SPLIT, OPT_SBR_LOOKAHEAD, OPT_NO_WINO43, OPT_NO_WINO43H, OPT_NO_PAIRS, OPT_PAIRS_MIN_TILES, OPT_NO_FUSED_ATTN, OPT_NO_WINO1D, OPT_NO_FUSED_GN, OPT_NO_FUSED_GN_LOAD, OPT_NO_FUSED_GN_LOAD_2SRC, OPT_NO_FUSED_GN_FIR, OPT_NO_2SRC_LD, OPT_NO_UP2_SLIDE, OPT_UP2_SLIDE_MIN_RUN, OPT_COUNT };
 bool option(Option o);
 int option_value(Option o);
 
diff --git a/id-diff_amd/csrc/igemm.hip b/id-diff_amd/csrc/igemm.hip
--- a/id-diff_amd/csrc/igemm.hip
+++ b/id-diff_amd/csrc/igemm.hip
@@ -28,6 +28,8 @@
   uint32_t c_bytes, res_bytes;
   int buf_ep;
   const float *scale_a, *scale_b;
+  uint32_t a2_pitch_delta;
+  int ld2;
 };
 
 __device__ __forceinline__ float4 ldg4(const float *p) { return *reinterpret_cast<const float4 *>(p); }
@@ -272,10 +274,14 @@
   return __builtin_bit_cast(float4, v);
 }
 
-template <int BM, int BN, int WARPS_M, int WARPS_N, bool CONV, bool DBUF, int SPLIT>
-__global__ void __launch_bounds__(WARPS_M *WARPS_N * 64, (DBUF || SPLIT) ? 2 : 4)
+constexpr int FORM_LD2 = 4;
+template <int BM, int BN, int WARPS_M, int WARPS_N, bool CONV, bool DBUF, int FORM>
+__global__ void __launch_bounds__(WARPS_M *WARPS_N * 64, (DBUF || (FORM & 3)) ? 2 : 4)
 igemm_pipe_kernel(const IgemmParams p) {
+  constexpr int SPLIT = FORM & 3;
+  constexpr bool LD2 = (FORM & FORM_LD2) != 0;
   static_assert(!(SPLIT && DBUF), "the split form uses one LDS buffer");
+  static_assert(!(LD2 && CONV), "two sources: the linear form");
   constexpr int T = WARPS_M * WARPS_N * 64;
   constexpr int WTM = BM / WARPS_M, WTN = BN / WARPS_N;
   constexpr int TM = WTM / 32, TN = WTN / 32;
@@ -379,8 +385,16 @@
       const bool second = p.K1 > 0 && f_kt * BK >= p.K1;
       const __amdgpu_buffer_rsrc_t rS = second ? rA2 : rA;
       const uint32_t koff = (uint32_t)(f_kt * BK - (second ? p.K1 : 0)) * 4u;
-#pragma unroll
-      for (int i = 0; i < A_PER_T; ++i) a_reg[i] = buf_load4(rS, (a_mask[i] && kok) ? a_base[i] + koff : OOB);
+      if constexpr (LD2) {
+        const uint32_t dl = second ? p.a2_pitch_delta : 0u;
+        const uint32_t koff2 = koff + (uint32_t)(m0 + row_base) * dl;
+#pragma unroll
+        for (int i = 0; i < A_PER_T; ++i)
+          a_reg[i] = buf_load4(rS, (a_mask[i] && kok) ? a_base[i] + koff2 + (uint32_t)(i * ROW_STEP) * dl : OOB);
+      } else {
+#pragma unroll
+        for (int i = 0; i < A_PER_T; ++i) a_reg[i] = buf_load4(rS, (a_mask[i] && kok) ? a_base[i] + koff : OOB);
+      }
     }
 #pragma unroll
     for (int i = 0; i < B_PER_T; ++i) b_reg[i] = buf_load4(rB, (b_ok[i] && kok) ? b_base[i] + koffb : OOB);
@@ -786,7 +800,7 @@
   }
 }
 
-template <int BM, int BN, int WARPS_M, int WARPS_N, bool CONV, bool DBUF = true, int SPLIT = 0>
+template <int BM, int BN, int WARPS_M, int WARPS_N, bool CONV, bool DBUF = true, int SPLIT = 0, bool LD2 = false>
 int launch_pipe(IgemmParams &p, int batch, hipStream_t st) {
   p.tiles_m = idiff::ceil_div(p.M, BM);
   p.tiles_n = idiff::ceil_div(p.N, BN);
@@ -794,7 +808,7 @@
                                        : (size_t)(DBUF ? 2 : 1) * (BM + BN) * LDS_PITCH * sizeof(float);
   constexpr size_t patch_bytes = (size_t)WARPS_M * WARPS_N * 32 * (BN / WARPS_N) * sizeof(float);
   constexpr size_t lds_bytes = stage_bytes > patch_bytes ? stage_bytes : patch_bytes;
-  auto kern = igemm_pipe_kernel<BM, BN, WARPS_M, WARPS_N, CONV, DBUF, SPLIT>;
+  auto kern = igemm_pipe_kernel<BM, BN, WARPS_M, WARPS_N, CONV, DBUF, SPLIT + (LD2 ? FORM_LD2 : 0)>;
   if (lds_bytes > 64 * 1024) {
     static idiff::AttrGuard guard;
     const void *fn = reinterpret_cast<const void *>(kern);
@@ -873,6 +887,26 @@
       if (t == 128128) return vec ? launch_cfg<128, 128, 2, 2, false, true>(p, batch, st) : launch_cfg<128, 128, 2, 2, false, false>(p, batch, st);
       if (t == 128064) return vec ? launch_cfg<128, 64, 2, 2, false, true>(p, batch, st) : launch_cfg<128, 64, 2, 2, false, false>(p, batch, st);
       if (t == 64064) return vec ? launch_cfg<64, 64, 2, 2, false, true>(p, batch, st) : launch_cfg<64, 64, 2, 2, false, false>(p, batch, st);
+    }
+  } else if (c.family == FAM_PIPE && p.ld2) {
+    if constexpr (!CONV) {
+      switch (c.arith) {
+        case AR_SPLIT:
+          if (t == 128128) return launch_pipe<128, 128, 2, 2, false, false, 1, true>(p, batch, st);
+          if (t == 128032) return launch_pipe<128, 32, 4, 1, false, false, 1, true>(p, batch, st);
+          if (t == 128064) return launch_pipe<128, 64, 2, 2, false, false, 1, true>(p, batch, st);
+          if (t == 64064) return launch_pipe<64, 64, 2, 2, false, false, 1, true>(p, batch, st);
+          break;
+        case AR_FP32_1BUF:
+          if (t == 128128) return launch_pipe<128, 128, 2, 2, false, false, 0, true>(p, batch, st);
+          break;
+        case AR_FP32:
+          if (t == 128128) return launch_pipe<128, 128, 2, 2, false, true, 0, true>(p, batch, st);
+          if (t == 128032) return launch_pipe<128, 32, 4, 1, false, true, 0, true>(p, batch, st);
+          if (t == 128064) return launch_pipe<128, 64, 2, 2, false, true, 0, true>(p, batch, st);
+          if (t == 64064) return launch_pipe<64, 64, 2, 2, false, true, 0, true>(p, batch, st);
+          break;
+      }
     }
   } else if (c.family == FAM_PIPE) {
     switch (c.arith) {
@@ -921,12 +955,14 @@
 
 enum PipeServes { PIPE_NO, PIPE_YES, PIPE_A_BEYOND };
 bool pitches16(int K, int64_t lda, int64_t ldb) { return K % 4 == 0 && lda % 4 == 0 && ldb % 4 == 0; }
-int pipe_fits_linear(int M, int N, int K, int64_t lda, int64_t ldb, int K1 = 0) {
-  if (!pitches16(K, lda, ldb) || extent_bytes(N, ldb, K) >= BUF_LIMIT) return PIPE_NO;
+int pipe_fits_linear(int M, int N, int K, int64_t lda, int64_t ldb, int K1 = 0, int64_t lda2 = 0) {
+  if (!pitches16(K, lda, ldb) || lda2 % 4 || extent_bytes(N, ldb, K) >= BUF_LIMIT) return PIPE_NO;
+  if (lda2 > 0)
+    return extent_bytes(M, lda, K1) < BUF_LIMIT && extent_bytes(M, lda2, K - K1) < BUF_LIMIT ? PIPE_YES : PIPE_A_BEYOND;
   return extent_bytes(M, lda, K1 > K - K1 ? K1 : K - K1) < BUF_LIMIT ? PIPE_YES : PIPE_A_BEYOND;
 }
-int pipe_serves_linear(int M, int N, int K, int64_t lda, int64_t ldb, int K1 = 0) {
-  return idiff::option(idiff::OPT_NO_PIPE) ? PIPE_NO : pipe_fits_linear(M, N, K, lda, ldb, K1);
+int pipe_serves_linear(int M, int N, int K, int64_t lda, int64_t ldb, int K1 = 0, int64_t lda2 = 0) {
+  return idiff::option(idiff::OPT_NO_PIPE) ? PIPE_NO : pipe_fits_linear(M, N, K, lda, ldb, K1, lda2);
 }
 int pipe_serves_conv(int B, int H, int W, int Cin, int Cout, int KH, int KW) {
   const int64_t K = (int64_t)KH * KW * Cin;
@@ -1044,6 +1080,7 @@
   int want;
   const float *w_scale, *act_scale;
   int weight_is_a;
+  int64_t lda2;
 };
 
 int linear_front(const LinearCall &c, hipStream_t st, IgemmPlan *probe) {
@@ -1055,20 +1092,23 @@
   if (c.M == 0 || c.N == 0 || c.batch == 0) { if (probe) probe->family = -1; return 0; }
   if (!c.A || (c.two_src && !c.A2) || !c.Bt || !c.C || (pairs && !c.w_scale)) return fail("%s: null pointer", c.name);
   if (c.K1 % BK) return fail("%s: the split column K1 = %d must be a multiple of %d", c.name, c.K1, BK);
-  if (c.lda < c.K1 || c.lda < c.K - c.K1 || c.ldb < c.K || c.ldc < c.N) return fail("%s: leading dimension smaller than the row length", c.name);
+  if (c.lda2 && (c.K - c.K1) % BK) return fail("%s: the second source's width K - K1 = %d must be a multiple of %d", c.name, c.K - c.K1, BK);
+  const int64_t lda2 = c.lda2 ? c.lda2 : c.lda;
+  if (c.lda2 < 0 || c.lda < c.K1 || lda2 < c.K - c.K1 || c.ldb < c.K || c.ldc < c.N)
+    return fail("%s: leading dimension smaller than the row length", c.name);
   if (pairs && !pairs_geometry_ok(c.M, c.N, c.K, c.batch))
     return fail("%s: M=%d N=%d K=%d batch=%d not served (ask idiff_gemm_pairs_ok)", c.name, c.M, c.N, c.K, c.batch);
   if (c.batch > 65535) return fail("%s: batch %d exceeds grid.y", c.name, c.batch);
-  const bool vec = pitches16(c.K, c.lda, c.ldb) && c.strideA % 4 == 0 && c.strideB % 4 == 0 && aligned16(c.A) &&
+  const bool vec = pitches16(c.K, c.lda, c.ldb) && lda2 % 4 == 0 && c.strideA % 4 == 0 && c.strideB % 4 == 0 && aligned16(c.A) &&
                    (!c.two_src || aligned16(c.A2)) && aligned16(c.Bt);
-  const int serves = !vec ? PIPE_NO : (pairs ? pipe_fits_linear : pipe_serves_linear)(c.M, c.N, c.K, c.lda, c.ldb, c.K1);
+  const int serves = !vec ? PIPE_NO : (pairs ? pipe_fits_linear : pipe_serves_linear)(c.M, c.N, c.K, c.lda, c.ldb, c.K1, c.lda2);
   if (serves == PIPE_A_BEYOND && c.batch == 1 && !pairs) {
     if (colstats) return fail("%s: colstats is not available for operands beyond 4 GiB", c.name);
     if (const int64_t cut = host_cut_row(c.M, 1, c.ep))
       return run_cut(c.M, cut, c.ep, probe != nullptr, [&](int64_t r0, int64_t r1, const idiff_epilogue *e) {
         LinearCall h = c;
         h.A += r0 * c.lda; h.C += r0 * c.ldc; h.M = (int)(r1 - r0); h.ep = e;
-        if (c.two_src) h.A2 += r0 * c.lda;
+        if (c.two_src) h.A2 += r0 * lda2;
         h.strideA = h.strideB = h.strideC = 0;
         return linear_front(h, st, probe);
       });
@@ -1086,14 +1126,15 @@
   }
   if (pairs && colstats && c.batch != 1) return fail("%s: colstats only for unbatched problems", c.name);
   p.a_bytes = (uint32_t)extent_bytes(c.M, c.lda, c.two_src ? c.K1 : c.K); p.b_bytes = (uint32_t)extent_bytes(c.N, c.ldb, c.K);
-  if (c.two_src) { p.A2 = c.A2; p.K1 = c.K1; p.a2_bytes = (uint32_t)extent_bytes(c.M, c.lda, c.K - c.K1); }
+  if (c.two_src) { p.A2 = c.A2; p.K1 = c.K1; p.a2_bytes = (uint32_t)extent_bytes(c.M, lda2, c.K - c.K1); }
+  if (c.two_src && lda2 != c.lda) { p.ld2 = 1; p.a2_pitch_delta = (uint32_t)((lda2 - c.lda) * 4); }
   if (pairs) { p.scale_a = c.weight_is_a ? c.w_scale : c.act_scale; p.scale_b = c.weight_is_a ? c.act_scale : c.w_scale; }
   return igemm_run<false>(p, c.batch, c.want, st, probe);
 }
 
 LinearCall linear_call(const char *name, const float *A, int64_t lda, int64_t strideA, const float *Bt, int64_t ldb, int64_t strideB, float *C,
                        int64_t ldc, int64_t strideC, int M, int N, int K, int batch, const idiff_epilogue *ep, int want) {
-  return LinearCall{name, A, nullptr, 0, false, Bt, C, lda, ldb, ldc, strideA, strideB, strideC, M, N, K, batch, ep, want, nullptr, nullptr, 0};
+  return LinearCall{name, A, nullptr, 0, false, Bt, C, lda, ldb, ldc, strideA, strideB, strideC, M, N, K, batch, ep, want, nullptr, nullptr, 0, 0};
 }
 LinearCall linear_call_2src(const char *name, const float *A1, const float *A2, int64_t lda, int K1, const float *Bt, int64_t ldb, float *C,
                             int64_t ldc, int M, int N, int K, const idiff_epilogue *ep, int want) {
@@ -1121,6 +1162,31 @@
 IDIFF_API int idiff_gemm_2src_f32(const float *A1, const float *A2, int64_t lda, int K1, const float *Bt, int64_t ldb,
                                   float *C, int64_t ldc, int M, int N, int K, const idiff_epilogue *ep, void *stream) {
   return linear_front(linear_call_2src("gemm_2src", A1, A2, lda, K1, Bt, ldb, C, ldc, M, N, K, ep, WANT_PIPE), (hipStream_t)stream, nullptr);
+}
+
+IDIFF_API int idiff_gemm_2src_ld_f32(const float *A1, int64_t lda1, int K1, const float *A2, int64_t lda2, int K2, const float *Bt, int64_t ldb,
+                                     float *C, int64_t ldc, int M, int N, const idiff_epilogue *ep, void *stream) {
+  if (K1 <= 0 || K2 <= 0 || lda2 <= 0) return idiff::fail("gemm_2src_ld: bad sizes K1=%d K2=%d lda2=%lld", K1, K2, (long long)lda2);
+  LinearCall c = linear_call_2src("gemm_2src_ld", A1, A2, lda1, K1, Bt, ldb, C, ldc, M, N, K1 + K2, ep, WANT_PIPE);
+  c.lda2 = lda2;
+  return linear_front(c, (hipStream_t)stream, nullptr);
+}
+
+IDIFF_API int idiff_gemm_2src_ld_ok(int M, int N, int K1, int K2, int64_t lda1, int64_t lda2, int64_t ldb) {
+  if (idiff::option(idiff::OPT_NO_2SRC_LD) || M <= 0 || N <= 0 || K1 <= 0 || K2 <= 0 || K1 % BK || K2 % BK) return 0;
+  if (lda1 < K1 || lda2 < K2 || ldb < (int64_t)K1 + K2) return 0;
+  return pipe_serves_linear(M, N, K1 + K2, lda1, ldb, K1, lda2) == PIPE_YES ? 1 : 0;
+}
+
+IDIFF_API const char *idiff_gemm_2src_ld_route(const void *A1, int64_t lda1, int K1, const void *A2, int64_t lda2, int K2, const void *Bt,
+                                               int64_t ldb, const void *C, int64_t ldc, int M, int N, const idiff_epilogue *ep) {
+  if (K1 <= 0 || K2 <= 0 || lda2 <= 0) { idiff::fail("gemm_2src_ld: bad sizes K1=%d K2=%d lda2=%lld", K1, K2, (long long)lda2); return nullptr; }
+  IgemmPlan plan = {};
+  LinearCall c = linear_call_2src("gemm_2src_ld", (const float *)A1, (const float *)A2, lda1, K1, (const float *)Bt, ldb,
+                                  (float *)const_cast<void *>(C), ldc, M, N, K1 + K2, ep, WANT_PIPE);
+  c.lda2 = lda2;
+  if (linear_front(c, nullptr, &plan)) return nullptr;
+  return plan.family < 0 ? "none" : igemm_plan_name(plan);
 }
 
 IDIFF_API int idiff_gemm_pairs_2src_f32(const float *A1, const float *A2, int64_t lda, int K1, const float *act_scale, const float *Bt,
diff --git a/id-diff_amd/csrc/runtime.hip b/id-diff_amd/csrc/runtime.hip
--- a/id-diff_amd/csrc/runtime.hip
+++ b/id-diff_amd/csrc/runtime.hip
@@ -17,7 +17,7 @@
                                              "IDIFF_DBUF_ONLY", "IDIFF_TRIDIAG_ONESTAGE", "IDIFF_UFD_ROWS", "IDIFF_CHASE_WAVEFRONT",
                                              "IDIFF_WINO_NGROUP", "IDIFF_GRAM_SMALL_TILES", "IDIFF_CHASE_SPIN_LIMIT",
                                              "IDIFF_FAKE_CU_COUNT", "IDIFF_SBR_SYNC", "IDIFF_SBR_FULL", "IDIFF_NO_SPLIT", "IDIFF_WINO_SPLIT", "IDIFF_SBR_LOOKAHEAD",
-                                             "IDIFF_NO_WINO43", "IDIFF_NO_WINO43H", "IDIFF_NO_PAIRS", "IDIFF_PAIRS_MIN_TILES", "IDIFF_NO_FUSED_ATTN", "IDIFF_NO_WINO1D", "IDIFF_NO_FUSED_GN", "IDIFF_NO_FUSED_GN_LOAD", "IDIFF_NO_FUSED_GN_LOAD_2SRC", "IDIFF_NO_FUSED_GN_FIR"};
+                                             "IDIFF_NO_WINO43", "IDIFF_NO_WINO43H", "IDIFF_NO_PAIRS", "IDIFF_PAIRS_MIN_TILES", "IDIFF_NO_FUSED_ATTN", "IDIFF_NO_WINO1D", "IDIFF_NO_FUSED_GN", "IDIFF_NO_FUSED_GN_LOAD", "IDIFF_NO_FUSED_GN_LOAD_2SRC", "IDIFF_NO_FUSED_GN_FIR", "IDIFF_NO_2SRC_LD", "IDIFF_NO_UP2_SLIDE", "IDIFF_UP2_SLIDE_MIN_RUN"};
 struct OptionTable {
   int v[OPT_COUNT];
   OptionTable() {
diff --git a/id-diff_amd/csrc/upfirdn2d.hip b/id-diff_amd/csrc/upfirdn2d.hip
--- a/id-diff_amd/csrc/upfirdn2d.hip
+++ b/id-diff_amd/csrc/upfirdn2d.hip
@@ -568,6 +568,7 @@
   }
 }
 
+constexpr int UFD_NO_NORM = -2;
 template <int ACT>
 __global__ void __launch_bounds__(256)
 upfirdn2d_nhwc_up2_block_gn(const float *__restrict__ x, const float *__restrict__ k, const float *__restrict__ coef,
@@ -585,8 +586,11 @@
   float w[16];
 #pragma unroll
   for (int t = 0; t < 16; ++t) w[t] = __builtin_bit_cast(float, __builtin_amdgcn_readfirstlane(__builtin_bit_cast(int, taps[t])));
-  const float4 *cp = reinterpret_cast<const float4 *>(coef) + ((int64_t)plane * cv + c4) * 2;
-  const float4 c01 = cp[0], c23 = cp[1];
+  float4 c01, c23;
+  if constexpr (ACT != UFD_NO_NORM) {
+    const float4 *cp = reinterpret_cast<const float4 *>(coef) + ((int64_t)plane * cv + c4) * 2;
+    c01 = cp[0]; c23 = cp[1];
+  }
   const float4 *xp = reinterpret_cast<const float4 *>(x) + (int64_t)plane * p.in_h * p.in_w * cv + c4;
   float4 *op = reinterpret_cast<float4 *>(out) + ((int64_t)plane * p.out_h + 2 * i) * p.out_w * cv + c4;
   const float4 zero = make_float4(0.f, 0.f, 0.f, 0.f);
@@ -602,7 +606,10 @@
     row[r] = xp + (int64_t)(vy[r] ? iy : 0) * p.in_w * cv;
   }
   auto raw = [&](int r, int ix) { return row[r][(int64_t)((unsigned)ix < (unsigned)p.in_w ? ix : 0) * cv]; };
-  auto normed = [&](int r, int ix, const float4 v) { return (vy[r] && (unsigned)ix < (unsigned)p.in_w) ? gn_act4<ACT>(v, c01, c23) : zero; };
+  auto normed = [&](int r, int ix, const float4 v) {
+    if constexpr (ACT == UFD_NO_NORM) return (vy[r] && (unsigned)ix < (unsigned)p.in_w) ? v : zero;
+    else return (vy[r] && (unsigned)ix < (unsigned)p.in_w) ? gn_act4<ACT>(v, c01, c23) : zero;
+  };
   float4 in[3][3];
 #pragma unroll
   for (int r = 0; r < 3; ++r) {
@@ -732,8 +739,14 @@
   int tx_log2;
   int toh, tow, tih, tiw, tiles_x;
   int cv, col_step;
+  bool slide;
   int64_t total;
 };
+
+bool up2_slide_routed(int in_w, int col_step) {
+  const int want = idiff::option_value(idiff::OPT_UP2_SLIDE_MIN_RUN);
+  return !idiff::option(idiff::OPT_NO_UP2_SLIDE) && (in_w + col_step - 1) / col_step >= (want > 0 ? want : 2);
+}
 
 int ufd_choose(const void *x, const void *out, int major, int in_h, int in_w, int minor, int kh, int kw, int up_x, int up_y,
                int down_x, int down_y, int pad_x0, int pad_x1, int pad_y0, int pad_y1, UfdParams &p, UfdPlan &c) {
@@ -824,6 +837,7 @@
     if (up_x == 2 && up_y == 2 && down_x == 1 && down_y == 1 && kh == 4 && kw == 4 && pad_x0 == 2 && pad_y0 == 2 &&
         p.out_h == 2 * in_h && p.out_w == 2 * in_w && (int64_t)major * in_h <= kMaxRowGroups && !option(OPT_UFD_ROWS)) {
       c.route = UFD_NHWC_UP2_BLOCK; c.grid = dim3(major * in_h);
+      c.slide = up2_slide_routed(in_w, c.col_step);
       return 0;
     }
     const int uplog = (up_x == up_y && kh <= 4 && kw <= 4) ? (up_x == 1 ? 0 : up_x == 2 ? 1 : -1) : -1;
@@ -890,6 +904,10 @@
       hipLaunchKernelGGL(upfirdn2d_planes_lds, c.grid, blk, c.lds, st, x, k, out, p, c.toh, c.tow, c.tih, c.tiw, c.ppb, c.tiles_x);
       return launch_status("upfirdn2d_planes_lds");
     case UFD_NHWC_UP2_BLOCK:
+      if (c.slide) {
+        hipLaunchKernelGGL(upfirdn2d_nhwc_up2_block_gn<UFD_NO_NORM>, c.grid, blk, 0, st, x, k, (const float *)nullptr, out, p, c.cv, c.col_step);
+        return launch_status("upfirdn2d_nhwc_up2_block_gn<no norm>");
+      }
       hipLaunchKernelGGL(upfirdn2d_nhwc_up2_block, c.grid, blk, 0, st, x, k, out, p, c.cv, c.col_step);
       return launch_status("upfirdn2d_nhwc_up2_block");
     case UFD_NHWC_ROWS0:
diff --git a/id-diff_amd/models/beatgans.py b/id-diff_amd/models/beatgans.py
--- a/id-diff_amd/models/beatgans.py
+++ b/id-diff_amd/models/beatgans.py
@@ -183,10 +183,16 @@
         if isinstance(mod.skip_connection, nn.Identity):
             sc = x if x2 is None else self._cat(x, x2)
         else:
-            split = x.C if x2 is not None else None
+            fused_ld = (x2 is not None and x.C % 32 == 0 and x2.C % 32 == 0 and
+                        _lib.gemm_2src_ld_ok(x.buf.shape[0] * x.H * x.W, mod.out_channels, x.C, x2.C))
+            split = x.C if (x2 is not None and not fused_ld) else None
             ws, bsk = self._cw(pk, mod.skip_connection, split)
             if x2 is None:
                 sc = self._pointwise(x, ws.view(ws.shape[0], -1), bsk)
+            elif fused_ld:
+                sc = self._new(x.buf.shape[0], x.H, x.W, ws.shape[0], x.buf)
+                _lib.gemm_2src_ld(x.buf.view(-1, x.C), x2.buf.view(-1, x2.C), ws.view(ws.shape[0], -1), sc.buf.view(-1, ws.shape[0]),
+                                  epilogue=_lib.make_epilogue(bias=bsk))
             else:
                 part = self._pointwise(x, ws[0].view(ws[0].shape[0], -1), bsk)
                 sc = self._pointwise(x2, ws[1].view(ws[1].shape[0], -1), None, residual=part.buf)
diff --git a/id-diff_amd/models/ncsnpp.py b/id-diff_amd/models/ncsnpp.py
--- a/id-diff_amd/models/ncsnpp.py
+++ b/id-diff_amd/models/ncsnpp.py
@@ -332,12 +332,14 @@
                               next_cout=mod.out_ch)
         if hasattr(mod, "Conv_2") or hasattr(mod, "NIN_0"):
             fused = x2 is not None and x.C == x2.C and x.C % 32 == 0
-            split = x.C if (x2 is not None and not fused) else None
+            fused_ld = (x2 is not None and not fused and x.C % 32 == 0 and x2.C % 32 == 0 and
+                        _lib.gemm_2src_ld_ok(x.buf.shape[0] * x.H * x.W, mod.out_ch, x.C, x2.C))
+            split = x.C if (x2 is not None and not fused and not fused_ld) else None
             if hasattr(mod, "Conv_2"):
-                ws, bs = self._conv_w(pk, (idx, 2), mod.Conv_2, split)
+                ws, bs = self._conv_w(pk, (idx, 2) if split is None else (idx, 2, split), mod.Conv_2, split)
                 ws = [w.view(w.shape[0], -1) for w in ws] if split is not None else ws.view(ws.shape[0], -1)
             else:
-                ws, bs = self._nin_w(pk, (idx, "nin"), mod.NIN_0, split)
+                ws, bs = self._nin_w(pk, (idx, "nin") if split is None else (idx, "nin", split), mod.NIN_0, split)
             if early_shortcut:
                 sc = resample(self._pointwise(x, ws, None))
             elif x2 is None:
@@ -346,6 +348,10 @@
                 sc = self._new(x.buf.shape[0], x.H, x.W, ws.shape[0], x.buf)
                 _lib.gemm_2src(x.buf.view(-1, x.C), x2.buf.view(-1, x2.C), ws, sc.buf.view(-1, ws.shape[0]),
                                epilogue=_lib.make_epilogue(bias=bs))
+            elif fused_ld:
+                sc = self._new(x.buf.shape[0], x.H, x.W, ws.shape[0], x.buf)
+                _lib.gemm_2src_ld(x.buf.view(-1, x.C), x2.buf.view(-1, x2.C), ws, sc.buf.view(-1, ws.shape[0]),
+                                  epilogue=_lib.make_epilogue(bias=bs))
             else:
                 part = self._pointwise(x, ws[0], bs)
                 sc = self._pointwise(x2, ws[1], None, residual=part.buf)
diff --git a/include/idiff_hip.h b/include/idiff_hip.h
--- a/include/idiff_hip.h
+++ b/include/idiff_hip.h
@@ -82,6 +82,12 @@
 
 int idiff_gemm_2src_f32(const float *A1, const float *A2, int64_t lda, int K1, const float *Bt, int64_t ldb, float *C,
                         int64_t ldc, int M, int N, int K, const idiff_epilogue *ep, void *stream);
+
+int idiff_gemm_2src_ld_f32(const float *A1, int64_t lda1, int K1, const float *A2, int64_t lda2, int K2, const float *Bt, int64_t ldb, float *C,
+                           int64_t ldc, int M, int N, const idiff_epilogue *ep, void *stream);
+int idiff_gemm_2src_ld_ok(int M, int N, int K1, int K2, int64_t lda1, int64_t lda2, int64_t ldb);
+const char *idiff_gemm_2src_ld_route(const void *A1, int64_t lda1, int K1, const void *A2, int64_t lda2, int K2, const void *Bt, int64_t ldb,
+                                     const void *C, int64_t ldc, int M, int N, const idiff_epilogue *ep);
 
 int idiff_conv2d_nhwc_f32(const float *x, const float *wt, float *out, int B, int H, int W, int Cin, int Cout,
                           int KH, int KW, int stride, int pad_lo, int pad_hi, const idiff_epilogue *ep, void *stream);
```

Measured after the change: 19180 (median of 6 runs). No clear change (+0.5%).
